# gooey-audio/libgooey

Measured on NVIDIA B200. Metric: voice-samples/sec, higher is better.
Workload: dtype f32

## Files before the change

### libgooey_b200/csrc/coop.cuh

```cuda
#pragma once
#include <climits>
#include <type_traits>
#include "wave.cuh"

namespace gd { namespace coop {
using namespace gd::wave;

constexpr unsigned FULL = 0xffffffffu;
constexpr int SP = 33;
enum { M_IDLE = 0, M_NORMAL = 1, M_TAIL = 2, M_GENERIC = 3, M_SERIAL = 4 };
enum { F_NORMAL = 1u << M_NORMAL, F_TAIL = 1u << M_TAIL, F_GENERIC = 1u << M_GENERIC, F_SERIAL = 1u << M_SERIAL, F_MEMBRANE = 1u << 8 };
struct RoundInfo { int j, nl, nv, mode; };
struct Empty {};

template <class C, int NV> struct Smem {
  typename std::conditional<C::GEO, GeoTables, Empty>::type T;
  typename C::V::Aud aud[NV];
  typename C::V::Run run[NV];
  typename C::Span2 w2[NV];
  RoundInfo ri[NV];
  unsigned wflags[2][NV];
  Lin2 lin[C::NLIN > 0 ? NV : 1][C::NLIN > 0 ? C::NLIN : 1];
  float st[C::NST][NV][SP];
};

__device__ __forceinline__ int warp_max(int x) {
#pragma unroll
  for (int d = 16; d > 0; d >>= 1) x = max(x, __shfl_xor_sync(FULL, x, d));
  return x;
}

struct TomC {
  using V = TomV;
  struct Span2 { int dummy; };
  static constexpr bool GEO = false;
  static constexpr int NLIN = 0;
  static constexpr int NST = 12;
  enum { ST_INC = 0, ST_FFWD = 0, ST_RND = 1, ST_A1 = 1, ST_FF = 2, ST_A2 = 2, ST_TP = 3, ST_FILT = 3, ST_FSP = 4, ST_RIN = 4, ST_RV = 5, ST_Y0 = 5,
         ST_ENV = 10, ST_NOISE = 11, ST_RLEV = 11 };
  static constexpr int MIN_CTAS = 2;
  static __device__ __forceinline__ int active_end(const TomV::Run&) { return 0x7fffffff; }
  template <class SM> static __device__ __forceinline__ void span_setup(SM&, int, int, const RateCtx&) {}

  template <int NV, class SM>
  static __device__ __forceinline__ void round(SM& S, const int warp, const int lane, const bool work, const float* p, const int j, int& nout, float& y,
                                               const RateCtx& rc, const unsigned rnd_idx) {
    TomAud& a = S.aud[warp];
    const TomV::Run& r = S.run[warp];
    const TomDer& d = r.d;
    const float sr = rc.sr;
    float (*st)[NV][SP] = S.st;
    const int nl = nout;
    int mode = M_IDLE, nv = 0;
    float env_l = 0.0f, noise_l = 0.0f, fade = 1.0f, mf_l = 40.0f, click = 0.0f;
    const unsigned le = (2u << lane) - 1u;
    if (work) {
      env_l = (j + lane) < r.j_env ? p[0] : r.env_final;
      noise_l = p[1];
      const float rnd_l = p[2];
      const bool complete_l = (j + lane) >= r.j_env;
      const unsigned valid = nl >= 32 ? FULL : ((1u << nl) - 1u);
      const float eb = env_l * d.bend_scaled;
      const float raw_freq = d.base_frequency * (1.0f + eb * eb);
      const unsigned m_att = __ballot_sync(FULL, env_l > 0.9f) & valid;
      const bool past0 = a.past_attack != 0u, done0 = a.main_done != 0u;
      const float ring0 = a.ring_level;
      const bool merged = a.tri_phase == a.main_sine_phase && a.tri_phase == a.mtri_phase && a.tri_phase == a.gated_sine_phase;
      const uint32_t cp = a.click_pos; const bool playing = a.click_playing != 0u;
      const bool past_l = past0 || (m_att & le) != 0u;
      const unsigned m_done = __ballot_sync(FULL, complete_l || (past_l && raw_freq < 20.0f)) & valid;
      const int first_done = done0 ? 0 : (m_done ? __ffs(m_done) - 1 : 32);
      __syncwarp();
      if (first_done == 0) {
        if (d.membrane > 0.0f && j >= r.j_env) {
          mode = M_TAIL; nv = nl;
          if (lane == 0) {
            a.main_done = 1;
            const float eb0 = r.env_final * d.bend_scaled;
            const float ff = fmaxf(fmaxf(d.base_frequency * (1.0f + eb0 * eb0), 40.0f), 20.0f);
            bp_set(a.bp, sr, ff, d.fq, 1.1f);
          }
        } else if (!(d.membrane > 0.0f) && !(ring0 > 0.0001f)) {
          mode = M_IDLE; nv = 0;
          if (lane == 0) { a.main_done = 1; a.active = 0; if (m_att & 1u) a.past_attack = 1; }
        } else { mode = M_GENERIC; nv = nl; }
      } else if (!merged) { mode = M_GENERIC; nv = nl; }
      else {
        mode = M_NORMAL; nv = first_done < nl ? first_done : nl;
        fade = (past_l && raw_freq < 40.0f) ? (raw_freq - 20.0f) / (40.0f - 20.0f) : 1.0f;
        mf_l = fmaxf(raw_freq, 40.0f);
        if (playing) { const uint32_t idx = cp + (uint32_t)lane; if (idx < 64u) click = c_tom_impulse[idx]; }
        if (lane == 0) {
          if ((m_att & (nv >= 32 ? FULL : ((1u << nv) - 1u))) != 0u) a.past_attack = 1;
          if (playing) { const uint32_t c2 = min(64u, cp + (uint32_t)nv); a.click_pos = c2; if (c2 >= 64u) a.click_playing = 0; }
        }
        st[ST_INC][warp][lane] = mf_l / sr;
        st[ST_FF][warp][lane] = fmaxf(mf_l, 20.0f);
      }
      if (mode == M_NORMAL || mode == M_GENERIC) st[ST_RND][warp][lane] = rnd_l;
      if (mode == M_GENERIC) { st[ST_ENV][warp][lane] = env_l; st[ST_NOISE][warp][lane] = noise_l; }
      if (lane == 0) {
        S.ri[warp].nv = nv; S.ri[warp].mode = mode;
      }
    }
    if (lane == 0) S.wflags[rnd_idx & 1u][warp] = mode == M_IDLE ? 0u : ((1u << mode) | ((d.membrane > 0.0f && mode != M_GENERIC) ? F_MEMBRANE : 0u));
    __syncthreads();
    const unsigned fl = __reduce_or_sync(FULL, lane < NV ? S.wflags[rnd_idx & 1u][lane] : 0u);
    if (fl & (F_NORMAL | F_GENERIC)) {
      if (warp == 0 && (fl & F_NORMAL)) {
        const int vv = lane < NV ? lane : 0;
        const bool on = lane < NV && S.ri[vv].mode == M_NORMAL;
        const int n_v = on ? S.ri[vv].nv : 0;
        TomAud& b = S.aud[vv];
        float ph = b.tri_phase, fx = b.fixed_sine_phase, rph = b.rand_phase, rcu = b.rand_current, rtg = b.rand_target;
        const float inc_fixed = 190.0f / sr, inc_rand = S.run[vv].d.rand_freq / sr;
        const float fq = S.run[vv].d.fq;
        float lf = b.bp.last_freq;
        bool qg_ok = fabsf(fq - b.bp.last_q) < 0.001f && fabsf(1.1f - b.bp.last_gain) < 0.001f;
        unsigned mask = 0u;
        const int nmax = warp_max(n_v);
        const float* r_inc = &st[ST_INC][vv][0]; const float* r_rnd = &st[ST_RND][vv][0]; const float* r_ff = &st[ST_FF][vv][0];
        float* w_tp = &st[ST_TP][vv][0]; float* w_fsp = &st[ST_FSP][vv][0]; float* w_rv = &st[ST_RV][vv][0];
        for (int n0 = 0; n0 < nmax; n0 += 8) {
          float inc[8], rnd[8], ffn[8];
#pragma unroll
          for (int k = 0; k < 8; k++) { inc[k] = r_inc[n0 + k]; rnd[k] = r_rnd[n0 + k]; ffn[k] = r_ff[n0 + k]; }
#pragma unroll
          for (int k = 0; k < 8; k++) {
            if (n0 + k < n_v) {
              w_tp[n0 + k] = ph; w_fsp[n0 + k] = fx;
              ph += inc[k]; if (ph >= 1.0f) ph -= 1.0f;
              fx += inc_fixed; if (fx >= 1.0f) fx -= 1.0f;
              const float prev = rph;
              rph += inc_rand; if (rph >= 1.0f) rph -= 1.0f;
              const bool wrap = rph < prev;
              rcu = wrap ? rtg : rcu; rtg = wrap ? rnd[k] : rtg;
              w_rv[n0 + k] = rcu + (rtg - rcu) * rph;
              const bool upd = !(fabsf(ffn[k] - lf) < 0.01f && qg_ok);
              lf = upd ? ffn[k] : lf; qg_ok = qg_ok || upd;
              mask |= upd ? (1u << (n0 + k)) : 0u;
            }
          }
        }
        if (on) {
          b.tri_phase = b.main_sine_phase = b.mtri_phase = b.gated_sine_phase = ph;
          b.fixed_sine_phase = fx; b.rand_phase = rph; b.rand_current = rcu; b.rand_target = rtg;
          b.bp.last_freq = lf;
          if (mask) { b.bp.last_q = fq; b.bp.last_gain = 1.1f; }
          S.ri[vv].nl = (int)mask;
        }
      }
      if (warp == (NV > 1 ? 1 : 0) && (fl & F_GENERIC)) {
        const int vv = lane < NV ? lane : 0;
        if (lane < NV && S.ri[vv].mode == M_GENERIC) {
          TomAud& b = S.aud[vv];
          const TomV::Run& rr = S.run[vv];
          const int jv = S.ri[vv].j, n_v = S.ri[vv].nv;
          int got = n_v;
          for (int n = 0; n < n_v; n++) {
            TomFront f; f.env = st[ST_ENV][vv][n]; f.noise = st[ST_NOISE][vv][n]; f.rnd = st[ST_RND][vv][n];
            const float yy = tom_back(b, rr.d, f, (jv + n) >= rr.j_env, rc);
            st[ST_TP][vv][n] = yy;
            if (!b.active) { got = n + 1; break; }
          }
          S.ri[vv].nv = got;
        }
      }
      __syncthreads();
    }
    float filtered = 0.0f;
    if (fl & F_NORMAL) {
      if (mode == M_NORMAL) {
        const float tp = st[ST_TP][warp][lane], fsp = st[ST_FSP][warp][lane], rand_value = st[ST_RV][warp][lane];
        const float ffl = st[ST_FF][warp][lane];
        const unsigned mask = (unsigned)S.ri[warp].nl;
        const float click_out = click * 1.1f;
        const float tri_out = a.tri_enabled ? tri_wave(tp) * 0.5f : 0.0f;
        const float us = unit_sine(tp);
        const float main_sine = us * 0.5f;
        const float mtri = tri_wave(tp) * 0.5f;
        const float fixed_sine = unit_sine(fsp) * 0.5f;
        const float noise = noise_l * 0.2f;
        const float noise_combined = (noise + rand_value) * 0.4f;
        const float gated = d.tone < 99.0f ? us * 0.2f : 0.0f;
        const float ch1 = main_sine * fixed_sine, ch2 = mtri + noise_combined, ch3 = noise_combined + gated;
        const float morph_out = ch1 * d.w1 + ch2 * d.w2 + ch3 * d.w3;
        const float x = click_out + tri_out + morph_out;
        float b0 = a.bp.b0, b1 = a.bp.b1, b2 = a.bp.b2, a1 = a.bp.a1, a2 = a.bp.a2;
        const float x1c = a.bp.x1, x2c = a.bp.x2;
        if (mask) {
          Biquad spec;
          bp_compute(spec, sr, ffl, d.fq, 1.1f);
          const unsigned m = mask & le;
          const int src = m ? 31 - __clz(m) : 0;
          const float sb0 = __shfl_sync(FULL, spec.b0, src), sb1 = __shfl_sync(FULL, spec.b1, src), sb2 = __shfl_sync(FULL, spec.b2, src);
          const float sa1 = __shfl_sync(FULL, spec.a1, src), sa2 = __shfl_sync(FULL, spec.a2, src);
          if (m) { b0 = sb0; b1 = sb1; b2 = sb2; a1 = sa1; a2 = sa2; }
        }
        float xm1 = __shfl_up_sync(FULL, x, 1), xm2 = __shfl_up_sync(FULL, x, 2);
        if (lane == 0) { xm1 = x1c; xm2 = x2c; } else if (lane == 1) xm2 = x1c;
        const float ffwd = b0 * x + b1 * xm1 + b2 * xm2;
        __syncwarp();
        st[ST_FFWD][warp][lane] = ffwd; st[ST_A1][warp][lane] = a1; st[ST_A2][warp][lane] = a2;
        if (lane == nv - 1) { Biquad& o = a.bp; o.b0 = b0; o.b1 = b1; o.b2 = b2; o.a1 = a1; o.a2 = a2; o.x1 = x; o.x2 = xm1; }
      }
      __syncthreads();
      if (warp == 0) {
        const int vv = lane < NV ? lane : 0;
        const bool on = lane < NV && S.ri[vv].mode == M_NORMAL;
        const int n_v = on ? S.ri[vv].nv : 0;
        float y1 = S.aud[vv].bp.y1, y2 = S.aud[vv].bp.y2;
        const int nmax = warp_max(n_v);
        const float* r_f = &st[ST_FFWD][vv][0]; const float* r_a1 = &st[ST_A1][vv][0]; const float* r_a2 = &st[ST_A2][vv][0];
        float* w_y = &st[ST_FILT][vv][0];
        for (int n0 = 0; n0 < nmax; n0 += 8) {
          float f[8], c1[8], c2[8], o[8];
#pragma unroll
          for (int k = 0; k < 8; k++) { f[k] = r_f[n0 + k]; c1[k] = r_a1[n0 + k]; c2[k] = r_a2[n0 + k]; }
#pragma unroll
          for (int k = 0; k < 8; k++) {
            o[k] = 0.0f;
            if (n0 + k < n_v) {
              const float out = f[k] - c1[k] * y1 - c2[k] * y2;
              y2 = y1; y1 = out;
              o[k] = fabsf(out) < 1e-15f ? 0.0f : out;
            }
          }
#pragma unroll
          for (int k = 0; k < 8; k++) if (n0 + k < n_v) w_y[n0 + k] = o[k];
        }
        if (on) { S.aud[vv].bp.y1 = y1; S.aud[vv].bp.y2 = y2; }
      }
      __syncthreads();
      if (mode == M_NORMAL) filtered = st[ST_FILT][warp][lane];
    }
    float mem_out = 0.0f, rlev = 0.0f;
    if (fl & F_MEMBRANE) {
      if ((mode == M_NORMAL || mode == M_TAIL) && d.membrane > 0.0f) {
        const float mi = mode == M_NORMAL ? filtered * env_l : 0.0f;
        const float u1 = __shfl_up_sync(FULL, mi, 1), u2 = __shfl_up_sync(FULL, mi, 2);
        float ffw[5], xp[5];
#pragma unroll
        for (int f = 0; f < 5; f++) {
          const Biquad& m = a.mem[f];
          const float xm1 = lane == 0 ? m.x1 : u1, xm2 = lane == 0 ? m.x2 : (lane == 1 ? m.x1 : u2);
          ffw[f] = m.b0 * mi + m.b1 * xm1 + m.b2 * xm2;
          xp[f] = xm1;
        }
        __syncwarp();
#pragma unroll
        for (int f = 0; f < 5; f++) {
          st[ST_Y0 + f][warp][lane] = ffw[f];
          if (lane == nv - 1) { a.mem[f].x1 = mi; a.mem[f].x2 = xp[f]; }
        }
      }
      __syncthreads();
      {
        const int q = warp * 32 + lane;
        const int f = q / NV, vv = q - f * NV;
        if (f < 5) {
          const int m = S.ri[vv].mode;
          const bool on = (m == M_NORMAL || m == M_TAIL) && S.run[vv].d.membrane > 0.0f;
          const int n_v = on ? S.ri[vv].nv : 0;
          const Biquad& bq = S.aud[vv].mem[f];
          const float a1 = bq.a1, a2 = bq.a2;
          float y1 = bq.y1, y2 = bq.y2;
          float* row = &st[ST_Y0 + f][vv][0];
          for (int n0 = 0; n0 < n_v; n0 += 8) {
            float in[8], o[8];
#pragma unroll
            for (int k = 0; k < 8; k++) in[k] = row[n0 + k];
#pragma unroll
            for (int k = 0; k < 8; k++) {
              o[k] = 0.0f;
              if (n0 + k < n_v) {
                const float out = in[k] - a1 * y1 - a2 * y2;
                y2 = y1; y1 = out;
                o[k] = fabsf(out) < 1e-15f ? 0.0f : out;
              }
            }
#pragma unroll
            for (int k = 0; k < 8; k++) if (n0 + k < n_v) row[n0 + k] = o[k];
          }
          if (on) { Biquad& o = S.aud[vv].mem[f]; o.y1 = y1; o.y2 = y2; }
        }
      }
      __syncthreads();
      if ((mode == M_NORMAL || mode == M_TAIL) && d.membrane > 0.0f) {
        float acc = 0.0f;
#pragma unroll
        for (int i = 0; i < 5; i++) acc += st[ST_Y0 + i][warp][lane];
        mem_out = w_tanh(acc);
        st[ST_RIN][warp][lane] = fabsf(mem_out) * 0.001f;
      }
      __syncthreads();
      if (warp == NV - 1) {
        const int vv = lane < NV ? lane : 0;
        const int m = S.ri[vv].mode;
        const bool on = lane < NV && (m == M_NORMAL || m == M_TAIL) && S.run[vv].d.membrane > 0.0f;
        const int n_v = on ? S.ri[vv].nv : 0;
        float ring = S.aud[vv].ring_level;
        if (m == M_TAIL) {
          int dead = -1;
          const float* r_in = &st[ST_RIN][vv][0]; float* w_lev = &st[ST_RLEV][vv][0];
          for (int n0 = 0; n0 < n_v && dead < 0; n0 += 8) {
            float in[8], lev[8];
#pragma unroll
            for (int k = 0; k < 8; k++) in[k] = r_in[n0 + k];
#pragma unroll
            for (int k = 0; k < 8; k++) {
              lev[k] = 0.0f;
              if (n0 + k < n_v && dead < 0) {
                if (!(ring > 0.0001f)) dead = n0 + k;
                else { ring = ring * 0.999f + in[k]; lev[k] = ring; }
              }
            }
#pragma unroll
            for (int k = 0; k < 8; k++) if (n0 + k < n_v) w_lev[n0 + k] = lev[k];
          }
          if (on && dead >= 0) { S.ri[vv].nv = dead; S.aud[vv].active = 0; }
        } else {
          const float* r_in = &st[ST_RIN][vv][0];
          for (int n0 = 0; n0 < n_v; n0 += 8) {
            float in[8];
#pragma unroll
            for (int k = 0; k < 8; k++) in[k] = r_in[n0 + k];
#pragma unroll
            for (int k = 0; k < 8; k++) if (n0 + k < n_v) ring = ring * 0.999f + in[k];
          }
        }
        if (on) S.aud[vv].ring_level = ring;
      }
      __syncthreads();
      if (mode == M_TAIL) rlev = st[ST_RLEV][warp][lane];
    }
    if (mode == M_NORMAL) {
      const float dry_gain = 1.0f - d.mm;
      const float dry = filtered * env_l;
      const float fs = dry * dry_gain + mem_out * d.mm;
      y = fs * fade * 0.7f * d.vol;
      nout = nv;
    } else if (mode == M_TAIL) {
      const float fd = rlev >= 0.005f ? 1.0f : (rlev <= 0.0001f ? 0.0f : (rlev - 0.0001f) / (0.005f - 0.0001f));
      y = mem_out * d.mm * fd * 0.7f * d.vol;
      nout = S.ri[warp].nv;
    } else if (mode == M_GENERIC) {
      y = st[ST_TP][warp][lane];
      nout = S.ri[warp].nv;
    } else nout = 0;
  }
};

template <class C, int NV>
__global__ void __launch_bounds__(NV * 32, C::MIN_CTAS) coop_kernel(const VoiceLaunch L) {
  using V = typename C::V; using Span = typename V::Span; using Aud = typename V::Aud;
  constexpr int WC = sizeof(typename V::Ctl) / 4;
  constexpr int WA = sizeof(Aud) / 4;
  extern __shared__ __align__(16) unsigned char coop_smem_raw[];
  Smem<C, NV>& S = *reinterpret_cast<Smem<C, NV>*>(coop_smem_raw);
  const int lane = threadIdx.x & 31, warp = threadIdx.x >> 5;
  if constexpr (C::GEO) geo_tables_init(S.T, L.rc, threadIdx.x, NV * 32);
  const int v = blockIdx.x * NV + warp;
  const bool alive = v < L.n && L.mode[v] == 0;
  const int sv = alive ? (L.slots ? (int)L.slots[v] : v) : 0;
  Aud& a = S.aud[warp];
  typename V::Run& run = S.run[warp];
  const Span* spans = nullptr;
  uint32_t ns = 0, cur = 0xffffffffu;
  bool ready = false;
  int next_j0 = 0x7fffffff;
  float* out = nullptr;
  const float* planes = nullptr;
  {
    uint32_t* aw = reinterpret_cast<uint32_t*>(&a);
    for (int w = lane; w < WA; w += 32) aw[w] = alive ? L.state[(size_t)(WC + w) * L.n_pad + sv] : 0u;
  }
  if (alive) {
    spans = reinterpret_cast<const Span*>(L.spans) + L.span_off[v];
    ns = L.n_spans[v];
    cur = L.span_cursor[v];
    if (cur != 0xffffffffu && lane == 0) V::span_resume(spans[cur], run);
    next_j0 = cur + 1u < ns ? spans[cur + 1u].j0 : 0x7fffffff;
    const long long row = L.rows ? (long long)L.rows[v] : (long long)(L.row0 + v);
    out = L.out + row * L.stride;
    planes = L.planes + (size_t)v * L.pitch;
  }
  if (lane == 0) S.ri[warp] = RoundInfo{0, 0, 0, M_IDLE};
  __syncthreads();
  const int c1 = L.chunk0 + min(L.chunk_frames, L.frames - L.chunk0);
  int j = L.chunk0;
  float pn[V::NPL];
  int pj = -1;
#pragma unroll
  for (int q = 0; q < V::NPL; q++) pn[q] = 0.0f;
  for (unsigned rnd_idx = 0;; rnd_idx++) {
    const bool more = alive && j < c1;
    bool work = false;
    int nl = 0;
    float p[V::NPL];
#pragma unroll
    for (int q = 0; q < V::NPL; q++) p[q] = 0.0f;
    if (more) {
      while (j == next_j0) {
        cur += 1u;
        if (lane == 0) V::span_begin(a, spans[cur], run, L.rc.sr);
        __syncwarp();
        ready = false;
        next_j0 = cur + 1u < ns ? spans[cur + 1u].j0 : 0x7fffffff;
      }
      const int span_end = min(next_j0, c1);
      const int act_end = min(span_end, C::active_end(run));
      if (cur == 0xffffffffu || !V::is_active(a, run, j) || j >= act_end) {
        for (int k = j + lane; k < span_end; k += 32) out[k] = 0.0f;
        j = span_end;
      } else {
        if (!ready) { __syncwarp(); C::span_setup(S, warp, lane, L.rc); __syncwarp(); ready = true; }
        nl = min(32, act_end - j);
        if (pj == j) {
#pragma unroll
          for (int q = 0; q < V::NPL; q++) { const float t = __shfl_sync(FULL, pn[q], nl - 1); p[q] = lane < nl ? pn[q] : t; }
        } else {
          const int jj = j + min(lane, nl - 1);
#pragma unroll
          for (int q = 0; q < V::NPL; q++) p[q] = planes[(size_t)q * L.plane_stride + (jj - L.chunk0)];
        }
        work = true;
        pj = j + nl;
        if (pj < c1) {
          const int jn = min(pj + lane, c1 - 1);
#pragma unroll
          for (int q = 0; q < V::NPL; q++) pn[q] = planes[(size_t)q * L.plane_stride + (jn - L.chunk0)];
        }
      }
    }
    __syncwarp();
    if (lane == 0) S.ri[warp] = RoundInfo{j, nl, nl, work ? M_NORMAL : M_IDLE};
    if (!__syncthreads_or(more ? 1 : 0)) break;
    float y = 0.0f;
    int nout = nl;
    C::template round<NV>(S, warp, lane, work, p, j, nout, y, L.rc, rnd_idx);
    if (work) {
      if (lane < nout) out[j + lane] = y;
      j += nout;
    }
  }
  __syncthreads();
  if (alive) {
    const uint32_t* aw = reinterpret_cast<const uint32_t*>(&a);
    for (int w = lane; w < WA; w += 32) L.state[(size_t)(WC + w) * L.n_pad + sv] = aw[w];
    if (lane == 0) L.span_cursor[v] = cur;
  }
}

} }
```

### libgooey_b200/csrc/gooey_b200.cu

```cuda
#include <mutex>
#include <memory>
#include "pool.cuh"
#include "patch.h"
#include "halfband_design.h"

namespace gh {

std::string& last_error() { static thread_local std::string e; return e; }
std::atomic<uint64_t> g_launches{0};
static float g_last_kernel_ms = 0.0f;
std::map<std::string, KernelStat>& kernel_stats() { static std::map<std::string, KernelStat> m; return m; }
std::mutex& kernel_stats_mutex() { static std::mutex m; return m; }

ClockTable& clock_table(float sr) {
  static std::mutex mu;
  static std::map<uint32_t, ClockTable*> tables;
  std::lock_guard<std::mutex> lk(mu);
  uint32_t key; memcpy(&key, &sr, 4);
  auto it = tables.find(key);
  if (it == tables.end()) {
    ClockTable* t = new ClockTable();
    t->dt = 1.0 / (double)sr;
    it = tables.emplace(key, t).first;
  }
  return *it->second;
}

static const int g_conn_env = setenv("CUDA_DEVICE_MAX_CONNECTIONS", "32", 0);

static std::mutex g_dev_mutex;
static std::vector<char> g_dev_ready;

static int device_count() {
  int n = 0;
  if (cudaGetDeviceCount(&n) != cudaSuccess) { cudaGetLastError(); return 0; }
  return n;
}

static void use_device(int device) {
  int n = device_count();
  if (n <= 0) throw CudaError("no CUDA device visible: libgooey_b200 has no CPU fallback");
  if (device < 0 || device >= n) throw CudaError("device index out of range");
  GH_CUDA(cudaSetDevice(device));
  std::lock_guard<std::mutex> lk(g_dev_mutex);
  if ((int)g_dev_ready.size() < n) g_dev_ready.resize(n, 0);
  if (!g_dev_ready[device]) {
    float hb[8];
    gd::design_halfband8(hb);
    GH_CUDA(cudaMemcpyToSymbol(gd::c_hb, hb, sizeof hb));
    {
      static float inv_sq[gd::INV_SQ_N];
      for (int k = 0; k < gd::INV_SQ_N; k++) { volatile float fi = (float)(2 * k + 1); volatile float sq = fi * fi; inv_sq[k] = 1.0f / sq; }
      GH_CUDA(cudaMemcpyToSymbol(gd::c_inv_sq, inv_sq, sizeof inv_sq));
    }
    double mf[128];
    for (int n = 0; n < 128; n++) mf[n] = 440.0 * pow(2.0, ((double)n - 69.0) / 12.0);
    GH_CUDA(cudaMemcpyToSymbol(gd::c_midi_freq, mf, sizeof mf));
    g_dev_ready[device] = 1;
  }
}

struct VoiceBank {
  TypeRunner<gd::KickV> kicks;
  TypeRunner<gd::SnareV> snares;
  TypeRunner<gd::HatV> hats;
  TypeRunner<gd::TomV> toms;
  TypeRunner<gd::BassV> basses;
  TypeRunner<gd::PolyV> polys;
  TypeRunner<gd::GranV> grans;
  void reset() { kicks.reset(); snares.reset(); hats.reset(); toms.reset(); basses.reset(); polys.reset(); grans.reset(); }
  int create(const GooeyVoicePatch& p, float sr) {
    switch (p.instrument) {
      case GOOEY_INSTRUMENT_KICK: { gd::KickState s; init_from_patch(s, p, sr); return kicks.pool.alloc(s); }
      case GOOEY_INSTRUMENT_SNARE: { gd::SnareState s; init_from_patch(s, p, sr); return snares.pool.alloc(s); }
      case GOOEY_INSTRUMENT_HIHAT: { gd::HatState s; init_from_patch(s, p, sr); return hats.pool.alloc(s); }
      case GOOEY_INSTRUMENT_TOM: { gd::TomState s; init_from_patch(s, p, sr); return toms.pool.alloc(s); }
      case GOOEY_INSTRUMENT_BASS: { gd::BassState s; init_from_patch(s, p, sr); return basses.pool.alloc(s); }
      case GOOEY_B200_VOICE_POLY: { gd::PolyState s; memset(&s, 0, sizeof s); gd::poly_init(s, p.params, sr); return polys.pool.alloc(s); }
      case GOOEY_B200_VOICE_GRANULATOR: { gd::GranState s; memset(&s, 0, sizeof s); gd::gran_init(s, sr); return grans.pool.alloc(s); }
      default: return -1;
    }
  }
  void set_mod(const float* planes, long long pitch, int frame0) {
    kicks.mod_planes = snares.mod_planes = hats.mod_planes = toms.mod_planes = basses.mod_planes = planes;
    kicks.mod_pitch = snares.mod_pitch = hats.mod_pitch = toms.mod_pitch = basses.mod_pitch = pitch;
    kicks.mod_frame0 = snares.mod_frame0 = hats.mod_frame0 = toms.mod_frame0 = basses.mod_frame0 = frame0;
  }
  void add(uint32_t type, uint32_t slot, uint32_t row, const std::vector<gd::VoiceEvent>& ev, const std::vector<gd::ModRoute>* routes = nullptr) {
    switch (type) {
      case GOOEY_INSTRUMENT_KICK: kicks.add(slot, row, ev, routes); break;
      case GOOEY_INSTRUMENT_SNARE: snares.add(slot, row, ev, routes); break;
      case GOOEY_INSTRUMENT_HIHAT: hats.add(slot, row, ev, routes); break;
      case GOOEY_INSTRUMENT_TOM: toms.add(slot, row, ev, routes); break;
      case GOOEY_INSTRUMENT_BASS: basses.add(slot, row, ev, routes); break;
      case GOOEY_B200_VOICE_POLY: polys.add(slot, row, ev); break;
      case GOOEY_B200_VOICE_GRANULATOR: grans.add(slot, row, ev); break;
    }
  }
  void release(uint32_t type, int slot) {
    switch (type) {
      case GOOEY_INSTRUMENT_KICK: kicks.pool.release(slot); break;
      case GOOEY_INSTRUMENT_SNARE: snares.pool.release(slot); break;
      case GOOEY_INSTRUMENT_HIHAT: hats.pool.release(slot); break;
      case GOOEY_INSTRUMENT_TOM: toms.pool.release(slot); break;
      case GOOEY_INSTRUMENT_BASS: basses.pool.release(slot); break;
      case GOOEY_B200_VOICE_POLY: polys.pool.release(slot); break;
      case GOOEY_B200_VOICE_GRANULATOR: grans.pool.release(slot); break;
    }
  }
  void launch(cudaStream_t parent, cudaEvent_t start, const gd::RateCtx& rc, const double* tt, int frames, float* out, long long stride) {
    kicks.launch(parent, start, rc, tt, frames, out, stride);
    snares.launch(parent, start, rc, tt, frames, out, stride);
    hats.launch(parent, start, rc, tt, frames, out, stride);
    toms.launch(parent, start, rc, tt, frames, out, stride);
    basses.launch(parent, start, rc, tt, frames, out, stride);
    polys.launch(parent, start, rc, tt, frames, out, stride);
    grans.launch(parent, start, rc, tt, frames, out, stride);
  }
  void collect_stats() { kicks.collect_stats(); snares.collect_stats(); hats.collect_stats(); toms.collect_stats(); }
  int chunk_frames(int frames) const { return TypeRunner<gd::KickV>::chunk_of(frames); }
  void wait_chunk(cudaStream_t s, int i) { kicks.wait_chunk(s, i); snares.wait_chunk(s, i); hats.wait_chunk(s, i); toms.wait_chunk(s, i); basses.wait_chunk(s, i); polys.wait_chunk(s, i); grans.wait_chunk(s, i); }
};

}

using namespace gh;

struct GooeyVoiceBatch {
  int device = 0;
  float sr = 44100.0f;
  gd::RateCtx rc;
  cudaStream_t stream = nullptr, copy_stream = nullptr;
  cudaEvent_t ev0 = nullptr, ev1 = nullptr;
  uint32_t n = 0;
  uint32_t k = 0;
  gh::ClockWindow clock;
  std::vector<uint8_t> vtype;
  std::vector<uint32_t> vslot;
  std::vector<std::vector<gd::VoiceEvent>> pending;
  VoiceBank bank;
  DevBuf<float> d_out;
  DevBuf<int16_t> d_pcm;
  ~GooeyVoiceBatch() {
    if (ev0) cudaEventDestroy(ev0);
    if (ev1) cudaEventDestroy(ev1);
    if (stream) cudaStreamDestroy(stream);
    if (copy_stream) cudaStreamDestroy(copy_stream);
  }
};

namespace gh {

static void voice_batch_render_impl(GooeyVoiceBatch* b, uint32_t frames, float* out_dev, size_t stride) {
  use_device(b->device);
  cudaStream_t st = b->stream;
  if ((uint64_t)b->k + frames >= 0xffffffffull) throw std::runtime_error("engine clock index overflow");
  const double* tt = b->clock.view(clock_table(b->sr), b->k, (uint64_t)b->k + frames, st);
  b->bank.reset();
  std::vector<gd::VoiceEvent> now, later;
  for (uint32_t v = 0; v < b->n; v++) {
    auto& ev = b->pending[v];
    std::stable_sort(ev.begin(), ev.end(), [](const gd::VoiceEvent& a, const gd::VoiceEvent& c) { return a.frame < c.frame; });
    now.clear(); later.clear();
    for (auto& e : ev) { if (e.frame < frames) now.push_back(e); else { e.frame -= frames; later.push_back(e); } }
    b->bank.add(b->vtype[v], b->vslot[v], v, now);
    ev = later;
  }
  GH_CUDA(cudaEventRecord(b->ev0, st));
  b->bank.launch(st, b->ev0, b->rc, tt, (int)frames, out_dev, (long long)stride);
  GH_CUDA(cudaEventRecord(b->ev1, st));
  b->k += frames;
}

}

#define GOOEY_TRY try {
#define GOOEY_CATCH                                                              \
  } catch (const gh::CudaError& e) { gh::set_error(e.what());                    \
    return std::string(e.what()).find("no CUDA device") != std::string::npos ? GOOEY_E_NO_DEVICE : GOOEY_E_CUDA; \
  } catch (const std::exception& e) { gh::set_error(e.what()); return GOOEY_E_INVALID; }

extern "C" {

const char* gooey_b200_last_error(void) { return gh::last_error().c_str(); }
int gooey_b200_device_count(void) { return gh::device_count(); }
uint64_t gooey_b200_launch_count(void) { return gh::g_launches.load(); }
float gooey_b200_last_kernel_ms(void) { return gh::g_last_kernel_ms; }
int gooey_b200_kernel_stat(const char* kernel, uint64_t* launches, double* total_ms, double* voice_frames) {
  if (!kernel) return GOOEY_E_INVALID;
  std::lock_guard<std::mutex> lk(gh::kernel_stats_mutex());
  auto it = gh::kernel_stats().find(kernel);
  gh::KernelStat k = it == gh::kernel_stats().end() ? gh::KernelStat() : it->second;
  if (launches) *launches = k.launches;
  if (total_ms) *total_ms = k.ms;
  if (voice_frames) *voice_frames = k.voice_frames;
  return GOOEY_E_OK;
}
const char* gooey_b200_kernel_stat_names(void) {
  static thread_local std::string names;
  std::lock_guard<std::mutex> lk(gh::kernel_stats_mutex());
  names.clear();
  for (const auto& kv : gh::kernel_stats()) { if (!names.empty()) names += ';'; names += kv.first; }
  return names.c_str();
}
void gooey_b200_kernel_stats_reset(void) { std::lock_guard<std::mutex> lk(gh::kernel_stats_mutex()); gh::kernel_stats().clear(); }

int gooey_voice_batch_new(float sample_rate, uint32_t n_voices, const GooeyVoicePatch* patches, int device, GooeyVoiceBatch** out_batch) {
  GOOEY_TRY
  if (!out_batch || (!patches && n_voices)) { set_error("null argument"); return GOOEY_E_INVALID; }
  *out_batch = nullptr;
  if (!(sample_rate > 0.0f)) { set_error("sample_rate must be > 0"); return GOOEY_E_INVALID; }
  use_device(device);
  std::unique_ptr<GooeyVoiceBatch> b(new GooeyVoiceBatch);
  b->device = device; b->sr = sample_rate; b->n = n_voices;
  b->rc = gd::make_rate_ctx(sample_rate);
  GH_CUDA(cudaStreamCreateWithFlags(&b->stream, cudaStreamNonBlocking));
  GH_CUDA(cudaStreamCreateWithFlags(&b->copy_stream, cudaStreamNonBlocking));
  GH_CUDA(cudaEventCreate(&b->ev0));
  GH_CUDA(cudaEventCreate(&b->ev1));
  b->vtype.resize(n_voices); b->vslot.resize(n_voices); b->pending.resize(n_voices);
  for (uint32_t v = 0; v < n_voices; v++) {
    int slot = b->bank.create(patches[v], sample_rate);
    if (slot < 0) { set_error("unsupported instrument id in voice patch"); return GOOEY_E_INVALID; }
    b->vtype[v] = (uint8_t)patches[v].instrument;
    b->vslot[v] = (uint32_t)slot;
  }
  *out_batch = b.release();
  return GOOEY_E_OK;
  GOOEY_CATCH
}

void gooey_voice_batch_free(GooeyVoiceBatch* b) {
  if (!b) return;
  cudaSetDevice(b->device);
  cudaDeviceSynchronize();
  delete b;
}

int gooey_voice_batch_trigger(GooeyVoiceBatch* b, uint32_t voice, uint32_t frame, float velocity) {
  GOOEY_TRY
  if (!b || voice >= b->n) { set_error("bad batch/voice"); return GOOEY_E_INVALID; }
  b->pending[voice].push_back(make_event(frame, gd::EV_TRIGGER, 0, velocity));
  return GOOEY_E_OK;
  GOOEY_CATCH
}

int gooey_voice_batch_trigger_all(GooeyVoiceBatch* b, uint32_t frame, const float* velocities) {
  GOOEY_TRY
  if (!b) { set_error("null batch"); return GOOEY_E_INVALID; }
  for (uint32_t v = 0; v < b->n; v++) b->pending[v].push_back(make_event(frame, gd::EV_TRIGGER, 0, velocities ? velocities[v] : 1.0f));
  return GOOEY_E_OK;
  GOOEY_CATCH
}

int gooey_voice_batch_set_param(GooeyVoiceBatch* b, uint32_t voice, uint32_t frame, uint32_t param, float value, int snap) {
  GOOEY_TRY
  if (!b || voice >= b->n) { set_error("bad batch/voice"); return GOOEY_E_INVALID; }
  bool known = ffi_param_to_events(b->vtype[voice], param, value,
                                   [&](uint32_t kind, uint32_t p, float v) { b->pending[voice].push_back(make_event(frame, kind, p, v)); });
  if (known && snap) b->pending[voice].push_back(make_event(frame, gd::EV_SNAP, 0, 0.0f));
  return GOOEY_E_OK;
  GOOEY_CATCH
}

int gooey_voice_batch_render_device(GooeyVoiceBatch* b, uint32_t frames, float* out_dev, size_t stride) {
  GOOEY_TRY
  if (!b || !out_dev || stride < frames) { set_error("bad arguments"); return GOOEY_E_INVALID; }
  voice_batch_render_impl(b, frames, out_dev, stride);
  GH_CUDA(cudaStreamSynchronize(b->stream));
  GH_CUDA(cudaEventElapsedTime(&gh::g_last_kernel_ms, b->ev0, b->ev1));
  b->bank.collect_stats();
  return GOOEY_E_OK;
  GOOEY_CATCH
}

int gooey_voice_batch_render(GooeyVoiceBatch* b, uint32_t frames, float* out_host) {
  GOOEY_TRY
  if (!b || !out_host) { set_error("bad arguments"); return GOOEY_E_INVALID; }
  use_device(b->device);
  const size_t stride = (frames + 3) & ~(size_t)3;
  b->d_out.alloc((size_t)b->n * stride);
  voice_batch_render_impl(b, frames, b->d_out.p, stride);
  const uint32_t chunk = (uint32_t)b->bank.chunk_frames((int)frames);
  int ci = 0;
  for (uint32_t c0 = 0; c0 < frames; c0 += chunk, ci++) {
    const uint32_t nf = std::min(chunk, frames - c0);
    b->bank.wait_chunk(b->copy_stream, ci);
    GH_CUDA(cudaMemcpy2DAsync(out_host + c0, (size_t)frames * 4, b->d_out.p + c0, stride * 4, (size_t)nf * 4, b->n, cudaMemcpyDeviceToHost, b->copy_stream));
  }
  GH_CUDA(cudaStreamSynchronize(b->copy_stream));
  GH_CUDA(cudaStreamSynchronize(b->stream));
  GH_CUDA(cudaEventElapsedTime(&gh::g_last_kernel_ms, b->ev0, b->ev1));
  b->bank.collect_stats();
  return GOOEY_E_OK;
  GOOEY_CATCH
}

}

#include "engine_api.cuh"
#include "rs_api.cuh"
#include "loops_api.cuh"
#include <sys/syscall.h>
#include <unistd.h>

extern "C" {

int gooey_voice_batch_render_pcm16(GooeyVoiceBatch* b, uint32_t frames, int16_t* out_host) {
  GOOEY_TRY
  if (!b || !out_host) { set_error("bad arguments"); return GOOEY_E_INVALID; }
  use_device(b->device);
  const size_t stride = (frames + 3) & ~(size_t)3;
  b->d_out.alloc((size_t)b->n * stride);
  b->d_pcm.alloc((size_t)b->n * stride);
  voice_batch_render_impl(b, frames, b->d_out.p, stride);
  const uint32_t chunk = (uint32_t)b->bank.chunk_frames((int)frames);
  int ci = 0;
  for (uint32_t c0 = 0; c0 < frames; c0 += chunk, ci++) {
    const uint32_t nf = std::min(chunk, frames - c0);
    b->bank.wait_chunk(b->copy_stream, ci);
    gd::quantize_pcm16_kernel<<<dim3((nf + 1023) / 1024, b->n), 256, 0, b->copy_stream>>>(b->d_out.p, (long long)stride, b->d_pcm.p, (long long)stride, (int)c0, (int)nf);
    g_launches.fetch_add(1, std::memory_order_relaxed);
    GH_CUDA(cudaGetLastError());
    GH_CUDA(cudaMemcpy2DAsync(out_host + c0, (size_t)frames * 2, b->d_pcm.p + c0, stride * 2, (size_t)nf * 2, b->n, cudaMemcpyDeviceToHost, b->copy_stream));
  }
  GH_CUDA(cudaStreamSynchronize(b->copy_stream));
  GH_CUDA(cudaStreamSynchronize(b->stream));
  GH_CUDA(cudaEventElapsedTime(&gh::g_last_kernel_ms, b->ev0, b->ev1));
  b->bank.collect_stats();
  return GOOEY_E_OK;
  GOOEY_CATCH
}

void* gooey_b200_host_alloc(size_t bytes, int device, int* out_numa_node) {
  if (out_numa_node) *out_numa_node = -1;
  if (bytes == 0) return nullptr;
  try { use_device(device); } catch (const std::exception& ex) { set_error(ex.what()); return nullptr; }
  int node = -1;
  char bus[32] = {0};
  if (cudaDeviceGetPCIBusId(bus, sizeof bus, device) == cudaSuccess) {
    for (char* c = bus; *c; c++) *c = (char)tolower(*c);
    const std::string path = std::string("/sys/bus/pci/devices/") + bus + "/numa_node";
    if (FILE* f = fopen(path.c_str(), "r")) { if (fscanf(f, "%d", &node) != 1) node = -1; fclose(f); }
  } else cudaGetLastError();
  bool bound = false;
#ifdef SYS_set_mempolicy
  if (node >= 0 && node < 1024) {
    unsigned long mask[16] = {0};
    mask[node / (8 * sizeof(unsigned long))] |= 1ul << (node % (8 * sizeof(unsigned long)));
    bound = syscall(SYS_set_mempolicy, 1 , mask, (unsigned long)(sizeof mask * 8)) == 0;
  }
#endif
  void* p = nullptr;
  const cudaError_t e = cudaHostAlloc(&p, bytes, cudaHostAllocPortable);
  if (e == cudaSuccess) memset(p, 0, bytes);
  if (e == cudaSuccess) {
    void* d = nullptr;
    const size_t chunk = (size_t)64 << 20;
    if (cudaMalloc(&d, std::min(chunk, bytes)) == cudaSuccess) {
      cudaMemset(d, 0, std::min(chunk, bytes));
      for (size_t off = 0; off < bytes; off += chunk)
        cudaMemcpyAsync((char*)p + off, d, std::min(chunk, bytes - off), cudaMemcpyDeviceToHost, 0);
      cudaDeviceSynchronize();
      cudaFree(d);
    }
    cudaGetLastError();
  }
#ifdef SYS_set_mempolicy
  if (bound) syscall(SYS_set_mempolicy, 0 , nullptr, 0ul);
#endif
  if (e != cudaSuccess) { cudaGetLastError(); set_error("cudaHostAlloc failed"); return nullptr; }
  if (out_numa_node) *out_numa_node = bound ? node : -1;
  return p;
}
void gooey_b200_host_free(void* p) { if (p) cudaFreeHost(p); }

}

namespace gh {
__global__ void math_selftest_kernel(int kind, const float* x, const float* y, float* out, uint32_t n) {
  uint32_t i = blockIdx.x * blockDim.x + threadIdx.x;
  if (i >= n) return;
  float r;
  switch (kind) {
    case 0: r = gm::g_powf(x[i], y[i]); break;
    case 1: r = gm::g_sinf(x[i]); break;
    case 2: r = gm::g_cosf(x[i]); break;
    case 3: r = gm::g_expf(x[i]); break;
    case 4: r = gd::hash_noise((uint64_t)x[i]); break;
    case 5: r = gd::max_curve(x[i], y[i]); break;
    case 6: r = gm::g_tanhf(x[i]); break;
    case 7: r = gm::g_tanf(x[i]); break;
    case 8: r = gm::g_expm1f(x[i]); break;
    case 9: r = gm::g_sinf_fast(x[i]); break;
    case 10: r = gm::g_div_by(x[i], y[i], 1.0f / y[i]); break;
    default: r = 0.0f;
  }
  out[i] = r;
}
}

extern "C" int gooey_b200_selftest_math(int kind, const float* x_host, const float* y_host, float* out_host, uint32_t n, int device) {
  GOOEY_TRY
  use_device(device);
  DevBuf<float> dx, dy, dout;
  dx.upload(x_host, n, 0);
  dy.upload(y_host ? y_host : x_host, n, 0);
  dout.alloc(n);
  gh::math_selftest_kernel<<<(n + 255) / 256, 256>>>(kind, dx.p, dy.p, dout.p, n);
  g_launches.fetch_add(1);
  GH_CUDA(cudaGetLastError());
  GH_CUDA(cudaMemcpy(out_host, dout.p, (size_t)n * 4, cudaMemcpyDeviceToHost));
  return GOOEY_E_OK;
  GOOEY_CATCH
}
```

### libgooey_b200/csrc/pool.cuh

```cuda
#pragma once
#include <algorithm>
#include <atomic>
#include <map>
#include <type_traits>
#include <set>
#include <mutex>
#include "device_rt.h"
#include "wave.cuh"
#include "coop.cuh"
#include "gran_wave.cuh"
#include "bass_wave.cuh"
#include "../../include/gooey_batch.h"

namespace gh {

extern std::atomic<uint64_t> g_launches;

struct KernelStat { uint64_t launches = 0; double ms = 0.0; double voice_frames = 0.0; };
std::map<std::string, KernelStat>& kernel_stats();
std::mutex& kernel_stats_mutex();

__global__ void scatter_words_kernel(uint32_t* __restrict__ dst, long long cap, const uint32_t* __restrict__ src, const uint32_t* __restrict__ slots,
                                     int n, int words) {
  const int k = blockIdx.x * blockDim.x + threadIdx.x;
  if (k >= n) return;
  const uint32_t s = slots[k];
  for (int w = 0; w < words; w++) dst[(long long)w * cap + s] = src[(long long)w * n + k];
}

template <class S> struct Pool {
  static_assert(sizeof(S) % 4 == 0, "state must be whole 32-bit words");
  static constexpr int W = sizeof(S) / 4;
  DevBuf<uint32_t> d;
  int cap = 0, count = 0;
  std::vector<int> free_list;
  std::vector<std::pair<int, S>> pending;

  int alloc(const S& init) {
    int slot;
    if (!free_list.empty()) { slot = free_list.back(); free_list.pop_back(); } else slot = count++;
    pending.emplace_back(slot, init);
    return slot;
  }
  void release(int slot) {
    for (size_t i = 0; i < pending.size(); i++) if (pending[i].first == slot) { pending.erase(pending.begin() + i); break; }
    free_list.push_back(slot);
  }
  void flush(cudaStream_t st) {
    if (count > cap) {
      int ncap = std::max(pad32(count), cap * 2);
      if (((ncap / 32) & 1) == 0) ncap += 32;
      DevBuf<uint32_t> nd;
      nd.alloc((size_t)W * ncap);
      GH_CUDA(cudaMemsetAsync(nd.p, 0, (size_t)W * ncap * 4, st));
      if (cap > 0) GH_CUDA(cudaMemcpy2DAsync(nd.p, (size_t)ncap * 4, d.p, (size_t)cap * 4, (size_t)cap * 4, W, cudaMemcpyDeviceToDevice, st));
      GH_CUDA(cudaStreamSynchronize(st));
      std::swap(d.p, nd.p); std::swap(d.n, nd.n);
      cap = ncap;
    }
    if (pending.empty()) return;
    const int n = (int)pending.size();
    std::vector<uint32_t> words((size_t)W * n), slots(n);
    for (int k = 0; k < n; k++) {
      slots[k] = (uint32_t)pending[k].first;
      const uint32_t* w = reinterpret_cast<const uint32_t*>(&pending[k].second);
      for (int i = 0; i < W; i++) words[(size_t)i * n + k] = w[i];
    }
    DevBuf<uint32_t> dw, ds;
    dw.upload(words.data(), words.size(), st);
    ds.upload(slots.data(), slots.size(), st);
    scatter_words_kernel<<<(n + 127) / 128, 128, 0, st>>>(d.p, cap, dw.p, ds.p, n, W);
    g_launches.fetch_add(1);
    GH_CUDA(cudaGetLastError());
    GH_CUDA(cudaStreamSynchronize(st));
    pending.clear();
    pending.shrink_to_fit();
  }
};

inline gd::VoiceEvent make_event(uint32_t frame, uint32_t kind, uint32_t param, float value, uint32_t aux = 0) {
  gd::VoiceEvent e; e.frame = frame; e.kind = (uint16_t)kind; e.param = (uint16_t)param; e.value = value; e.aux = aux;
  return e;
}

struct ClockTable {
  static constexpr uint64_t CK = 65536;
  double dt = 0.0;
  std::vector<double> ckpt;
  std::mutex mu;
  void fill(uint64_t k0, size_t n, double* out) {
    std::lock_guard<std::mutex> lk(mu);
    if (ckpt.empty()) ckpt.push_back(0.0);
    const uint64_t need = k0 / CK;
    while (ckpt.size() <= need) { double t = ckpt.back(); for (uint64_t i = 0; i < CK; i++) t += dt; ckpt.push_back(t); }
    double t = ckpt[need];
    for (uint64_t k = need * CK; k < k0; k++) t += dt;
    for (size_t i = 0; i < n; i++) { out[i] = t; t += dt; }
  }
};
struct ClockWindow {
  DevBuf<double> d;
  std::vector<double> h;
  uint64_t k0 = 0; size_t n = 0;
  const double* view(ClockTable& T, uint64_t kmin, uint64_t kmax, cudaStream_t st) {
    if (kmin > 0) kmin -= 1;
    if (!(n && kmin >= k0 && kmax < k0 + n)) {
      const size_t want = (size_t)(kmax - kmin + 1);
      const size_t cap = std::max<size_t>((want + 8191) & ~(size_t)8191, 1u << 16);
      if (d.n < cap) { GH_CUDA(cudaStreamSynchronize(st)); d.alloc(cap); }
      h.resize(want);
      T.fill(kmin, want, h.data());
      GH_CUDA(cudaMemcpyAsync(d.p, h.data(), want * sizeof(double), cudaMemcpyHostToDevice, st));
      GH_CUDA(cudaStreamSynchronize(st));
      k0 = kmin; n = want;
    }
    return d.p - k0;
  }
};
ClockTable& clock_table(float sr);

enum class Back { Wave, Coop, Serial };
constexpr int COOP_FROM = 4096;
constexpr int COOP_NV = 16;
constexpr int SERIAL_FROM = 12288;
inline bool serial_backend() { const char* e = getenv("GOOEY_B200_BACKEND"); return e && strcmp(e, "serial") == 0; }
template <class V> inline Back choose_back(int cnt) {
  if (serial_backend()) return Back::Serial;
  if (std::is_same<V, gd::TomV>::value) return cnt >= COOP_FROM ? Back::Coop : Back::Wave;
  return cnt >= SERIAL_FROM ? Back::Serial : Back::Wave;
}
template <class V> struct WaveOf;
template <> struct WaveOf<gd::KickV> { using W = gd::wave::KickW; static constexpr const char* name = "wave_kernel<KickW>"; };
template <> struct WaveOf<gd::SnareV> { using W = gd::wave::SnareW; static constexpr const char* name = "wave_kernel<SnareW>"; };
template <> struct WaveOf<gd::HatV> { using W = gd::wave::HatW; static constexpr const char* name = "wave_kernel<HatW>"; };
template <> struct WaveOf<gd::TomV> { using W = gd::wave::TomW; static constexpr const char* name = "wave_kernel<TomW>"; };

inline void coop_launch(int cnt, cudaStream_t s, const gd::VoiceLaunch& L) {
  using SM = gd::coop::Smem<gd::coop::TomC, COOP_NV>;
  auto kernel = gd::coop::coop_kernel<gd::coop::TomC, COOP_NV>;
  static std::mutex mu;
  static std::set<int> done;
  int dev = 0;
  cudaGetDevice(&dev);
  {
    std::lock_guard<std::mutex> lk(mu);
    if (done.insert(dev).second) {
      GH_CUDA(cudaFuncSetAttribute((const void*)kernel, cudaFuncAttributeMaxDynamicSharedMemorySize, (int)sizeof(SM)));
      GH_CUDA(cudaFuncSetAttribute((const void*)kernel, cudaFuncAttributePreferredSharedMemoryCarveout, (int)cudaSharedmemCarveoutMaxShared));
    }
  }
  kernel<<<(cnt + COOP_NV - 1) / COOP_NV, COOP_NV * 32, sizeof(SM), s>>>(L);
}

template <class K> inline void same_carveout(K kernel) {
  static std::mutex mu;
  static std::set<std::pair<int, const void*>> done;
  int dev = 0;
  cudaGetDevice(&dev);
  std::lock_guard<std::mutex> lk(mu);
  if (done.insert({dev, (const void*)kernel}).second)
    GH_CUDA(cudaFuncSetAttribute((const void*)kernel, cudaFuncAttributePreferredSharedMemoryCarveout, (int)cudaSharedmemCarveoutMaxShared));
}
#define GH_LAUNCH(kernel, grid, block, stream, ...) do { same_carveout(kernel); kernel<<<grid, block, 0, stream>>>(__VA_ARGS__); } while (0)

constexpr int CHUNK_FRAMES = 8192;
template <class V> struct TypeRunner {
  using State = typename V::State;
  Pool<State> pool;
  std::vector<uint32_t> slots, rows, ev_begin, span_off;
  std::vector<gd::VoiceEvent> ev_flat;
  std::vector<gd::ModRoute> routes_flat; std::vector<uint32_t> route_begin;
  DevBuf<gd::ModRoute> d_routes; DevBuf<uint32_t> d_route_begin;
  const float* mod_planes = nullptr; long long mod_pitch = 0; int mod_frame0 = 0;
  DevBuf<uint32_t> d_slots, d_rows, d_ev_begin, d_span_off, d_n_spans, d_span_cursor;
  DevBuf<gd::VoiceEvent> d_events;
  DevBuf<uint8_t> d_mode, d_spans;
  DevBuf<float> d_planes[2];
  cudaStream_t sB = nullptr, sC = nullptr, sS = nullptr;
  cudaEvent_t evA = nullptr, evB[2] = {nullptr, nullptr}, evC[2] = {nullptr, nullptr}, evDoneC = nullptr, evDoneS = nullptr;
  std::vector<cudaEvent_t> evT0, evT1;
  std::vector<double> timed_units;
  std::vector<cudaEvent_t> evChunk;
  int launched_chunks = 0;
  const char* backend_name = "back_kernel";
  static int chunk_of(int frames) { return std::min(CHUNK_FRAMES, (frames + 31) & ~31); }
  void wait_chunk(cudaStream_t s, int i) {
    if (n() == 0) return;
    if (launched_chunks == 0) { GH_CUDA(cudaStreamWaitEvent(s, evDoneC, 0)); return; }
    GH_CUDA(cudaStreamWaitEvent(s, evDoneS, 0));
    GH_CUDA(cudaStreamWaitEvent(s, evChunk[std::min(i, std::abs(launched_chunks) - 1)], 0));
  }

  int n() const { return (int)slots.size(); }
  void reset() { slots.clear(); rows.clear(); ev_flat.clear(); ev_begin.clear(); ev_begin.push_back(0); span_off.clear(); span_off.push_back(0);
                 routes_flat.clear(); route_begin.clear(); route_begin.push_back(0); }
  void add(uint32_t slot, uint32_t out_row, const std::vector<gd::VoiceEvent>& events, const std::vector<gd::ModRoute>* routes = nullptr) {
    slots.push_back(slot); rows.push_back(out_row);
    if (routes) routes_flat.insert(routes_flat.end(), routes->begin(), routes->end());
    route_begin.push_back((uint32_t)routes_flat.size());
    uint32_t distinct = 0, last = 0xffffffffu;
    for (const auto& e : events) { if (e.frame != last) { distinct++; last = e.frame; } }
    ev_flat.insert(ev_flat.end(), events.begin(), events.end());
    ev_begin.push_back((uint32_t)ev_flat.size());
    span_off.push_back(span_off.back() + distinct + 1);
  }
  void ensure_streams() {
    if (sC) return;
    GH_CUDA(cudaStreamCreateWithFlags(&sB, cudaStreamNonBlocking));
    GH_CUDA(cudaStreamCreateWithFlags(&sC, cudaStreamNonBlocking));
    GH_CUDA(cudaStreamCreateWithFlags(&sS, cudaStreamNonBlocking));
    cudaEvent_t* evs[] = {&evA, &evB[0], &evB[1], &evC[0], &evC[1], &evDoneC, &evDoneS};
    for (auto e : evs) GH_CUDA(cudaEventCreateWithFlags(e, cudaEventDisableTiming));
  }
  ~TypeRunner() {
    cudaEvent_t evs[] = {evA, evB[0], evB[1], evC[0], evC[1], evDoneC, evDoneS};
    for (auto e : evs) if (e) cudaEventDestroy(e);
    for (auto e : evChunk) cudaEventDestroy(e);
    for (auto e : evT0) cudaEventDestroy(e);
    for (auto e : evT1) cudaEventDestroy(e);
    if (sB) cudaStreamDestroy(sB);
    if (sC) cudaStreamDestroy(sC);
    if (sS) cudaStreamDestroy(sS);
  }
  void collect_stats() {
    const char* name = backend_name;
    if (launched_chunks <= 0) return;
    std::lock_guard<std::mutex> lk(kernel_stats_mutex());
    KernelStat& k = kernel_stats()[name];
    for (int i = 0; i < launched_chunks; i++) {
      float ms = 0.0f;
      if (cudaEventElapsedTime(&ms, evT0[i], evT1[i]) != cudaSuccess) { cudaGetLastError(); continue; }
      k.launches++; k.ms += ms; k.voice_frames += timed_units[i];
    }
    launched_chunks = -launched_chunks;
  }
  void launch(cudaStream_t parent, cudaEvent_t start, const gd::RateCtx& rc, const double* tt, int frames, float* out, long long stride) {
    const int cnt = n();
    launched_chunks = 0;
    if (cnt == 0 || frames <= 0) return;
    ensure_streams();
    GH_CUDA(cudaStreamWaitEvent(sC, start, 0));
    pool.flush(sC);
    d_slots.upload(slots.data(), slots.size(), sC);
    d_rows.upload(rows.data(), rows.size(), sC);
    if (ev_flat.empty()) ev_flat.push_back(make_event(0xffffffffu, 0xffff, 0, 0.0f));
    d_events.upload(ev_flat.data(), ev_flat.size(), sC);
    d_ev_begin.upload(ev_begin.data(), ev_begin.size(), sC);
    gd::VoiceLaunch L;
    memset(&L, 0, sizeof L);
    L.state = pool.d.p; L.n = cnt; L.n_pad = pool.cap;
    L.slots = d_slots.p; L.rows = d_rows.p; L.row0 = 0;
    L.events = d_events.p; L.ev_begin = d_ev_begin.p; L.tt = tt; L.frames = frames; L.out = out; L.stride = stride; L.rc = rc;
    const bool modulated = !routes_flat.empty() && mod_planes;
    if (modulated) {
      d_routes.upload(routes_flat.data(), routes_flat.size(), sC);
      d_route_begin.upload(route_begin.data(), route_begin.size(), sC);
      L.routes = d_routes.p; L.route_begin = d_route_begin.p; L.mod_planes = mod_planes; L.mod_pitch = mod_pitch; L.mod_frame0 = mod_frame0;
    }
    if constexpr (V::FAST) {
      using Span = typename V::Span;
      d_span_off.upload(span_off.data(), span_off.size(), sC);
      d_n_spans.alloc(cnt); d_span_cursor.alloc(cnt); d_mode.alloc(cnt);
      d_spans.alloc((size_t)span_off.back() * sizeof(Span));
      const int chunk = chunk_of(frames);
      const int rows_pad = pad32(cnt);
      const size_t plane_floats = (size_t)rows_pad * chunk;
      d_planes[0].alloc(plane_floats * V::NPL); d_planes[1].alloc(plane_floats * V::NPL);
      L.mode = d_mode.p; L.spans = d_spans.p; L.span_off = d_span_off.p; L.n_spans = d_n_spans.p; L.span_cursor = d_span_cursor.p;
      L.plane_stride = (long long)plane_floats; L.pitch = chunk;
      GH_LAUNCH((gd::plan_kernel<V>), (cnt + 63) / 64, 64, sC, L);
      g_launches.fetch_add(1, std::memory_order_relaxed);
      GH_CUDA(cudaGetLastError());
      GH_CUDA(cudaEventRecord(evA, sC));
      GH_CUDA(cudaStreamWaitEvent(sB, evA, 0));
      GH_CUDA(cudaStreamWaitEvent(sS, evA, 0));
      GH_LAUNCH((gd::slow_kernel<V, 32>), (cnt + 31) / 32, 32, sS, L);
      g_launches.fetch_add(1, std::memory_order_relaxed);
      GH_CUDA(cudaGetLastError());
      GH_CUDA(cudaEventRecord(evDoneS, sS));
      const Back back = choose_back<V>(cnt);
      int i = 0;
      for (int c0 = 0; c0 < frames; c0 += chunk, i++) {
        const int b = i & 1;
        L.chunk0 = c0; L.chunk_frames = std::min(chunk, frames - c0);
        L.planes = d_planes[b].p;
        if (i >= 2) GH_CUDA(cudaStreamWaitEvent(sB, evC[b], 0));
        const int bpv = (L.chunk_frames + 255) / 256;
        GH_LAUNCH((gd::front_kernel<V, 256>), (unsigned)((size_t)cnt * bpv), 256, sB, L, bpv);
        GH_CUDA(cudaGetLastError());
        GH_CUDA(cudaEventRecord(evB[b], sB));
        GH_CUDA(cudaStreamWaitEvent(sC, evB[b], 0));
        if ((int)evT0.size() <= i) { cudaEvent_t e0, e1; GH_CUDA(cudaEventCreate(&e0)); GH_CUDA(cudaEventCreate(&e1)); evT0.push_back(e0); evT1.push_back(e1); timed_units.push_back(0.0); }
        timed_units[i] = (double)cnt * L.chunk_frames;
        GH_CUDA(cudaEventRecord(evT0[i], sC));
        switch (back) {
          case Back::Coop:
            if constexpr (std::is_same<V, gd::TomV>::value) coop_launch(cnt, sC, L);
            backend_name = "coop_kernel<TomC>";
            break;
          case Back::Wave:
            GH_LAUNCH((gd::wave::wave_kernel<typename WaveOf<V>::W>), cnt, 32, sC, L);
            backend_name = WaveOf<V>::name;
            break;
          case Back::Serial:
            GH_LAUNCH((gd::back_kernel<V, 32>), (cnt + 31) / 32, 32, sC, L);
            backend_name = "back_kernel";
            break;
        }
        GH_CUDA(cudaGetLastError());
        GH_CUDA(cudaEventRecord(evT1[i], sC));
        GH_CUDA(cudaEventRecord(evC[b], sC));
        if ((int)evChunk.size() <= i) { cudaEvent_t e; GH_CUDA(cudaEventCreateWithFlags(&e, cudaEventDisableTiming)); evChunk.push_back(e); }
        GH_CUDA(cudaEventRecord(evChunk[i], sC));
        g_launches.fetch_add(2, std::memory_order_relaxed);
      }
      launched_chunks = i;
      GH_CUDA(cudaEventRecord(evDoneC, sC));
      GH_CUDA(cudaStreamWaitEvent(parent, evDoneC, 0));
      GH_CUDA(cudaStreamWaitEvent(parent, evDoneS, 0));
      if (getenv("GOOEY_B200_TRACE_TYPES")) {
        cudaEvent_t t0, t1, t2;
        cudaEventCreate(&t0); cudaEventCreate(&t1); cudaEventCreate(&t2);
        cudaEventRecord(t1, sC); cudaEventRecord(t2, sS);
        GH_CUDA(cudaStreamSynchronize(sC)); GH_CUDA(cudaStreamSynchronize(sS));
        std::vector<uint8_t> mode(cnt);
        GH_CUDA(cudaMemcpy(mode.data(), d_mode.p, cnt, cudaMemcpyDeviceToHost));
        int slow = 0; for (uint8_t m : mode) slow += m != 0;
        float ms_all = 0.0f;
        cudaEventElapsedTime(&ms_all, evT0[0], t1);
        float ms_slow_end = 0.0f;
        cudaEventElapsedTime(&ms_slow_end, evT0[0], t2);
        fprintf(stderr, "[gooey trace]   %s: %d voices x %d frames, %d on the per-sample path; back ends done %.1f ms, per-sample kernel done %.1f ms after the first back-end launch\n",
                backend_name, cnt, frames, slow, ms_all, ms_slow_end);
        cudaEventDestroy(t0); cudaEventDestroy(t1); cudaEventDestroy(t2);
      }
    } else {
      if constexpr (std::is_same<V, gd::GranV>::value) {
        GH_LAUNCH((gd::gran_wave_kernel<4>), (cnt + 3) / 4, 128, sC, L);
      } else if (std::is_same<V, gd::BassV>::value && !modulated) {
        const bool ttrace = getenv("GOOEY_B200_TRACE_TYPES") != nullptr;
        cudaEvent_t t0 = nullptr, t1 = nullptr;
        if (ttrace) { cudaEventCreate(&t0); cudaEventCreate(&t1); cudaEventRecord(t0, sC); }
        GH_LAUNCH((gd::bass_wave_kernel<2>), (cnt + 1) / 2, 64, sC, L);
        if (ttrace) {
          cudaEventRecord(t1, sC); GH_CUDA(cudaStreamSynchronize(sC));
          float ms = 0.0f; cudaEventElapsedTime(&ms, t0, t1);
          fprintf(stderr, "[gooey trace]   bass_wave_kernel: %d voices x %d frames, %.1f ms\n", cnt, frames, ms);
          cudaEventDestroy(t0); cudaEventDestroy(t1);
        }
      } else if (cnt <= 148 * 32 * 4) GH_LAUNCH((gd::slow_kernel<V, 32>), (cnt + 31) / 32, 32, sC, L);
      else GH_LAUNCH((gd::slow_kernel<V, 128>), (cnt + 127) / 128, 128, sC, L);
      g_launches.fetch_add(1, std::memory_order_relaxed);
      GH_CUDA(cudaGetLastError());
      GH_CUDA(cudaEventRecord(evDoneC, sC));
      GH_CUDA(cudaStreamWaitEvent(parent, evDoneC, 0));
    }
  }
};

}
```

Baseline: 8.403 billion.

## Pipeline tom coop kernel into multi-round staggered stages across specialized warps

Restructures the cooperative tom kernel from one synchronous round, where a few warps run serial recurrences while the others wait, into a software pipeline of depth four. Each stage runs on its own warp: phase/random, filter-update mask, bandpass recurrence, five membrane biquads and ring level, plus a dedicated generic warp. A ring buffer of round info lets each stage work on a different in-flight block. The voices per block drop from 16 to 8, and the coop backend is now chosen by the total drum voice count rather than the tom count alone. This adds shared-memory staging and pipeline fill/drain bookkeeping, with a risk of ordering bugs around generic and tail modes.

```diff
diff --git a/libgooey_b200/csrc/coop.cuh b/libgooey_b200/csrc/coop.cuh
--- a/libgooey_b200/csrc/coop.cuh
+++ b/libgooey_b200/csrc/coop.cuh
@@ -8,21 +8,10 @@
 
 constexpr unsigned FULL = 0xffffffffu;
 constexpr int SP = 33;
-enum { M_IDLE = 0, M_NORMAL = 1, M_TAIL = 2, M_GENERIC = 3, M_SERIAL = 4 };
-enum { F_NORMAL = 1u << M_NORMAL, F_TAIL = 1u << M_TAIL, F_GENERIC = 1u << M_GENERIC, F_SERIAL = 1u << M_SERIAL, F_MEMBRANE = 1u << 8 };
-struct RoundInfo { int j, nl, nv, mode; };
-struct Empty {};
-
-template <class C, int NV> struct Smem {
-  typename std::conditional<C::GEO, GeoTables, Empty>::type T;
-  typename C::V::Aud aud[NV];
-  typename C::V::Run run[NV];
-  typename C::Span2 w2[NV];
-  RoundInfo ri[NV];
-  unsigned wflags[2][NV];
-  Lin2 lin[C::NLIN > 0 ? NV : 1][C::NLIN > 0 ? C::NLIN : 1];
-  float st[C::NST][NV][SP];
-};
+constexpr int DEPTH = 4;
+constexpr int RING = 8;
+enum { M_IDLE = 0, M_NORMAL = 1, M_TAIL = 2, M_GENERIC = 3 };
+struct RoundInfo { int j, nl, nv, mode; unsigned mask; };
 
 __device__ __forceinline__ int warp_max(int x) {
 #pragma unroll
@@ -32,99 +21,52 @@
 
 struct TomC {
   using V = TomV;
-  struct Span2 { int dummy; };
-  static constexpr bool GEO = false;
-  static constexpr int NLIN = 0;
-  static constexpr int NST = 12;
-  enum { ST_INC = 0, ST_FFWD = 0, ST_RND = 1, ST_A1 = 1, ST_FF = 2, ST_A2 = 2, ST_TP = 3, ST_FILT = 3, ST_FSP = 4, ST_RIN = 4, ST_RV = 5, ST_Y0 = 5,
-         ST_ENV = 10, ST_NOISE = 11, ST_RLEV = 11 };
-  static constexpr int MIN_CTAS = 2;
-  static __device__ __forceinline__ int active_end(const TomV::Run&) { return 0x7fffffff; }
-  template <class SM> static __device__ __forceinline__ void span_setup(SM&, int, int, const RateCtx&) {}
+  static constexpr int NST = 18;
+  enum { ST_INC = 0, ST_ENV = 0, ST_RND = 1, ST_FF = 2, ST_NOISE = 2,
+         ST_TP = 3, ST_FSP = 4, ST_RV = 5,
+         ST_FFWD = 6, ST_A1 = 7, ST_A2 = 8,
+         ST_FILT = 9,
+         ST_Y0 = 10,
+         ST_RIN = 15,
+         ST_RLEV = 16,
+         ST_GEN = 17 };
+  enum { W_S1 = 0, W_S2 = 1, W_S3 = 2, W_S4 = 5, W_GEN = 6, W_S1M = 7 };
+  static constexpr int MIN_WARPS = 32;
+
+  template <int NV> struct Smem {
+    TomAud aud[NV];
+    TomV::Run run[NV];
+    RoundInfo ri[RING][NV];
+    int dead_j[NV];
+    float st[NST][NV][SP];
+  };
+  struct Carry {
+    float noise, click, ff, env, fade;
+    float env_c, fade_c;
+    float dry, fade_d;
+    float pre;
+  };
 
   template <int NV, class SM>
-  static __device__ __forceinline__ void round(SM& S, const int warp, const int lane, const bool work, const float* p, const int j, int& nout, float& y,
-                                               const RateCtx& rc, const unsigned rnd_idx) {
-    TomAud& a = S.aud[warp];
-    const TomV::Run& r = S.run[warp];
-    const TomDer& d = r.d;
+  static __device__ __forceinline__ void s_half(SM& S, const int warp, const int lane, const unsigned t, const RateCtx& rc) {
     const float sr = rc.sr;
     float (*st)[NV][SP] = S.st;
-    const int nl = nout;
-    int mode = M_IDLE, nv = 0;
-    float env_l = 0.0f, noise_l = 0.0f, fade = 1.0f, mf_l = 40.0f, click = 0.0f;
-    const unsigned le = (2u << lane) - 1u;
-    if (work) {
-      env_l = (j + lane) < r.j_env ? p[0] : r.env_final;
-      noise_l = p[1];
-      const float rnd_l = p[2];
-      const bool complete_l = (j + lane) >= r.j_env;
-      const unsigned valid = nl >= 32 ? FULL : ((1u << nl) - 1u);
-      const float eb = env_l * d.bend_scaled;
-      const float raw_freq = d.base_frequency * (1.0f + eb * eb);
-      const unsigned m_att = __ballot_sync(FULL, env_l > 0.9f) & valid;
-      const bool past0 = a.past_attack != 0u, done0 = a.main_done != 0u;
-      const float ring0 = a.ring_level;
-      const bool merged = a.tri_phase == a.main_sine_phase && a.tri_phase == a.mtri_phase && a.tri_phase == a.gated_sine_phase;
-      const uint32_t cp = a.click_pos; const bool playing = a.click_playing != 0u;
-      const bool past_l = past0 || (m_att & le) != 0u;
-      const unsigned m_done = __ballot_sync(FULL, complete_l || (past_l && raw_freq < 20.0f)) & valid;
-      const int first_done = done0 ? 0 : (m_done ? __ffs(m_done) - 1 : 32);
-      __syncwarp();
-      if (first_done == 0) {
-        if (d.membrane > 0.0f && j >= r.j_env) {
-          mode = M_TAIL; nv = nl;
-          if (lane == 0) {
-            a.main_done = 1;
-            const float eb0 = r.env_final * d.bend_scaled;
-            const float ff = fmaxf(fmaxf(d.base_frequency * (1.0f + eb0 * eb0), 40.0f), 20.0f);
-            bp_set(a.bp, sr, ff, d.fq, 1.1f);
-          }
-        } else if (!(d.membrane > 0.0f) && !(ring0 > 0.0001f)) {
-          mode = M_IDLE; nv = 0;
-          if (lane == 0) { a.main_done = 1; a.active = 0; if (m_att & 1u) a.past_attack = 1; }
-        } else { mode = M_GENERIC; nv = nl; }
-      } else if (!merged) { mode = M_GENERIC; nv = nl; }
-      else {
-        mode = M_NORMAL; nv = first_done < nl ? first_done : nl;
-        fade = (past_l && raw_freq < 40.0f) ? (raw_freq - 20.0f) / (40.0f - 20.0f) : 1.0f;
-        mf_l = fmaxf(raw_freq, 40.0f);
-        if (playing) { const uint32_t idx = cp + (uint32_t)lane; if (idx < 64u) click = c_tom_impulse[idx]; }
-        if (lane == 0) {
-          if ((m_att & (nv >= 32 ? FULL : ((1u << nv) - 1u))) != 0u) a.past_attack = 1;
-          if (playing) { const uint32_t c2 = min(64u, cp + (uint32_t)nv); a.click_pos = c2; if (c2 >= 64u) a.click_playing = 0; }
-        }
-        st[ST_INC][warp][lane] = mf_l / sr;
-        st[ST_FF][warp][lane] = fmaxf(mf_l, 20.0f);
-      }
-      if (mode == M_NORMAL || mode == M_GENERIC) st[ST_RND][warp][lane] = rnd_l;
-      if (mode == M_GENERIC) { st[ST_ENV][warp][lane] = env_l; st[ST_NOISE][warp][lane] = noise_l; }
-      if (lane == 0) {
-        S.ri[warp].nv = nv; S.ri[warp].mode = mode;
-      }
-    }
-    if (lane == 0) S.wflags[rnd_idx & 1u][warp] = mode == M_IDLE ? 0u : ((1u << mode) | ((d.membrane > 0.0f && mode != M_GENERIC) ? F_MEMBRANE : 0u));
-    __syncthreads();
-    const unsigned fl = __reduce_or_sync(FULL, lane < NV ? S.wflags[rnd_idx & 1u][lane] : 0u);
-    if (fl & (F_NORMAL | F_GENERIC)) {
-      if (warp == 0 && (fl & F_NORMAL)) {
-        const int vv = lane < NV ? lane : 0;
-        const bool on = lane < NV && S.ri[vv].mode == M_NORMAL;
-        const int n_v = on ? S.ri[vv].nv : 0;
-        TomAud& b = S.aud[vv];
+    const int vv = lane < NV ? lane : 0;
+    if (warp == W_S1 || warp == W_S1M) {
+      const RoundInfo& q = S.ri[(t - 1u) & (RING - 1)][vv];
+      const bool on = lane < NV && q.mode == M_NORMAL;
+      const int n_v = on ? q.nv : 0;
+      const int nmax = warp_max(n_v);
+      TomAud& b = S.aud[vv];
+      if (nmax > 0 && warp == W_S1) {
         float ph = b.tri_phase, fx = b.fixed_sine_phase, rph = b.rand_phase, rcu = b.rand_current, rtg = b.rand_target;
         const float inc_fixed = 190.0f / sr, inc_rand = S.run[vv].d.rand_freq / sr;
-        const float fq = S.run[vv].d.fq;
-        float lf = b.bp.last_freq;
-        bool qg_ok = fabsf(fq - b.bp.last_q) < 0.001f && fabsf(1.1f - b.bp.last_gain) < 0.001f;
-        unsigned mask = 0u;
-        const int nmax = warp_max(n_v);
-        const float* r_inc = &st[ST_INC][vv][0]; const float* r_rnd = &st[ST_RND][vv][0]; const float* r_ff = &st[ST_FF][vv][0];
+        const float* r_inc = &st[ST_INC][vv][0]; const float* r_rnd = &st[ST_RND][vv][0];
         float* w_tp = &st[ST_TP][vv][0]; float* w_fsp = &st[ST_FSP][vv][0]; float* w_rv = &st[ST_RV][vv][0];
         for (int n0 = 0; n0 < nmax; n0 += 8) {
-          float inc[8], rnd[8], ffn[8];
-#pragma unroll
-          for (int k = 0; k < 8; k++) { inc[k] = r_inc[n0 + k]; rnd[k] = r_rnd[n0 + k]; ffn[k] = r_ff[n0 + k]; }
+          float inc[8], rnd[8];
+#pragma unroll
+          for (int k = 0; k < 8; k++) { inc[k] = r_inc[n0 + k]; rnd[k] = r_rnd[n0 + k]; }
 #pragma unroll
           for (int k = 0; k < 8; k++) {
             if (n0 + k < n_v) {
@@ -136,6 +78,26 @@
               const bool wrap = rph < prev;
               rcu = wrap ? rtg : rcu; rtg = wrap ? rnd[k] : rtg;
               w_rv[n0 + k] = rcu + (rtg - rcu) * rph;
+            }
+          }
+        }
+        if (on) {
+          b.tri_phase = b.main_sine_phase = b.mtri_phase = b.gated_sine_phase = ph;
+          b.fixed_sine_phase = fx; b.rand_phase = rph; b.rand_current = rcu; b.rand_target = rtg;
+        }
+      } else if (nmax > 0) {
+        const float fq = S.run[vv].d.fq;
+        float lf = b.bp.last_freq;
+        bool qg_ok = fabsf(fq - b.bp.last_q) < 0.001f && fabsf(1.1f - b.bp.last_gain) < 0.001f;
+        unsigned mask = 0u;
+        const float* r_ff = &st[ST_FF][vv][0];
+        for (int n0 = 0; n0 < nmax; n0 += 8) {
+          float ffn[8];
+#pragma unroll
+          for (int k = 0; k < 8; k++) ffn[k] = r_ff[n0 + k];
+#pragma unroll
+          for (int k = 0; k < 8; k++) {
+            if (n0 + k < n_v) {
               const bool upd = !(fabsf(ffn[k] - lf) < 0.01f && qg_ok);
               lf = upd ? ffn[k] : lf; qg_ok = qg_ok || upd;
               mask |= upd ? (1u << (n0 + k)) : 0u;
@@ -143,44 +105,200 @@
           }
         }
         if (on) {
-          b.tri_phase = b.main_sine_phase = b.mtri_phase = b.gated_sine_phase = ph;
-          b.fixed_sine_phase = fx; b.rand_phase = rph; b.rand_current = rcu; b.rand_target = rtg;
           b.bp.last_freq = lf;
           if (mask) { b.bp.last_q = fq; b.bp.last_gain = 1.1f; }
-          S.ri[vv].nl = (int)mask;
-        }
-      }
-      if (warp == (NV > 1 ? 1 : 0) && (fl & F_GENERIC)) {
-        const int vv = lane < NV ? lane : 0;
-        if (lane < NV && S.ri[vv].mode == M_GENERIC) {
-          TomAud& b = S.aud[vv];
-          const TomV::Run& rr = S.run[vv];
-          const int jv = S.ri[vv].j, n_v = S.ri[vv].nv;
-          int got = n_v;
-          for (int n = 0; n < n_v; n++) {
-            TomFront f; f.env = st[ST_ENV][vv][n]; f.noise = st[ST_NOISE][vv][n]; f.rnd = st[ST_RND][vv][n];
-            const float yy = tom_back(b, rr.d, f, (jv + n) >= rr.j_env, rc);
-            st[ST_TP][vv][n] = yy;
-            if (!b.active) { got = n + 1; break; }
-          }
-          S.ri[vv].nv = got;
-        }
-      }
-      __syncthreads();
-    }
-    float filtered = 0.0f;
-    if (fl & F_NORMAL) {
-      if (mode == M_NORMAL) {
+          S.ri[(t - 1u) & (RING - 1)][vv].mask = mask;
+        }
+      }
+    } else if (warp == W_GEN) {
+      RoundInfo& q = S.ri[(t - 1u) & (RING - 1)][vv];
+      if (lane < NV && q.mode == M_GENERIC) {
+        TomAud& b = S.aud[vv];
+        const TomV::Run& rr = S.run[vv];
+        const int jv = q.j, n_v = q.nv;
+        int got = n_v;
+        for (int n = 0; n < n_v; n++) {
+          TomFront f; f.env = st[ST_ENV][vv][n]; f.noise = st[ST_NOISE][vv][n]; f.rnd = st[ST_RND][vv][n];
+          const float yy = tom_back(b, rr.d, f, (jv + n) >= rr.j_env, rc);
+          st[ST_GEN][vv][n] = yy;
+          if (!b.active) { got = n + 1; break; }
+        }
+        q.nv = got;
+      }
+    } else if (warp == W_S2) {
+      const RoundInfo& q = S.ri[(t - 2u) & (RING - 1)][vv];
+      const bool on = lane < NV && q.mode == M_NORMAL;
+      const int n_v = on ? q.nv : 0;
+      const int nmax = warp_max(n_v);
+      if (nmax > 0) {
+        float y1 = S.aud[vv].bp.y1, y2 = S.aud[vv].bp.y2;
+        const float* r_f = &st[ST_FFWD][vv][0]; const float* r_a1 = &st[ST_A1][vv][0]; const float* r_a2 = &st[ST_A2][vv][0];
+        float* w_y = &st[ST_FILT][vv][0];
+        for (int n0 = 0; n0 < nmax; n0 += 8) {
+          float f[8], c1[8], c2[8], o[8];
+#pragma unroll
+          for (int k = 0; k < 8; k++) { f[k] = r_f[n0 + k]; c1[k] = r_a1[n0 + k]; c2[k] = r_a2[n0 + k]; }
+#pragma unroll
+          for (int k = 0; k < 8; k++) {
+            o[k] = 0.0f;
+            if (n0 + k < n_v) {
+              const float out = f[k] - c1[k] * y1 - c2[k] * y2;
+              y2 = y1; y1 = out;
+              o[k] = fabsf(out) < 1e-15f ? 0.0f : out;
+            }
+          }
+#pragma unroll
+          for (int k = 0; k < 8; k++) if (n0 + k < n_v) w_y[n0 + k] = o[k];
+        }
+        if (on) { S.aud[vv].bp.y1 = y1; S.aud[vv].bp.y2 = y2; }
+      }
+    } else if (warp >= W_S3 && warp < W_S3 + 3) {
+      const int qi = (warp - W_S3) * 32 + lane;
+      const int f = qi / NV, v3 = qi - f * NV;
+      if (f < 5) {
+        const RoundInfo& q = S.ri[(t - 3u) & (RING - 1)][v3];
+        const bool on = (q.mode == M_NORMAL || q.mode == M_TAIL) && S.run[v3].d.membrane > 0.0f;
+        const int n_v = on ? q.nv : 0;
+        if (n_v > 0) {
+          Biquad& bq = S.aud[v3].mem[f];
+          const float a1 = bq.a1, a2 = bq.a2;
+          float y1 = bq.y1, y2 = bq.y2;
+          float* row = &st[ST_Y0 + f][v3][0];
+          for (int n0 = 0; n0 < n_v; n0 += 8) {
+            float in[8], o[8];
+#pragma unroll
+            for (int k = 0; k < 8; k++) in[k] = row[n0 + k];
+#pragma unroll
+            for (int k = 0; k < 8; k++) {
+              o[k] = 0.0f;
+              if (n0 + k < n_v) {
+                const float out = in[k] - a1 * y1 - a2 * y2;
+                y2 = y1; y1 = out;
+                o[k] = fabsf(out) < 1e-15f ? 0.0f : out;
+              }
+            }
+#pragma unroll
+            for (int k = 0; k < 8; k++) if (n0 + k < n_v) row[n0 + k] = o[k];
+          }
+          bq.y1 = y1; bq.y2 = y2;
+        }
+      }
+    } else if (warp == W_S4) {
+      RoundInfo& q = S.ri[(t - 4u) & (RING - 1)][vv];
+      const bool on = lane < NV && (q.mode == M_NORMAL || q.mode == M_TAIL) && S.run[vv].d.membrane > 0.0f && q.j < S.dead_j[vv];
+      const int n_v = on ? q.nv : 0;
+      if (n_v > 0) {
+        float ring = S.aud[vv].ring_level;
+        const float* r_in = &st[ST_RIN][vv][0];
+        if (q.mode == M_TAIL) {
+          int dead = -1;
+          float* w_lev = &st[ST_RLEV][vv][0];
+          for (int n0 = 0; n0 < n_v && dead < 0; n0 += 8) {
+            float in[8], lev[8];
+#pragma unroll
+            for (int k = 0; k < 8; k++) in[k] = r_in[n0 + k];
+#pragma unroll
+            for (int k = 0; k < 8; k++) {
+              lev[k] = 0.0f;
+              if (n0 + k < n_v && dead < 0) {
+                if (!(ring > 0.0001f)) dead = n0 + k;
+                else { ring = ring * 0.999f + in[k]; lev[k] = ring; }
+              }
+            }
+#pragma unroll
+            for (int k = 0; k < 8; k++) if (n0 + k < n_v) w_lev[n0 + k] = lev[k];
+          }
+          if (dead >= 0) { q.nv = dead; S.aud[vv].active = 0; S.dead_j[vv] = q.j + dead; }
+        } else {
+          for (int n0 = 0; n0 < n_v; n0 += 8) {
+            float in[8];
+#pragma unroll
+            for (int k = 0; k < 8; k++) in[k] = r_in[n0 + k];
+#pragma unroll
+            for (int k = 0; k < 8; k++) if (n0 + k < n_v) ring = ring * 0.999f + in[k];
+          }
+        }
+        S.aud[vv].ring_level = ring;
+      }
+    }
+  }
+
+  template <int NV, class SM>
+  static __device__ __forceinline__ void p_half(SM& S, const int warp, const int lane, const unsigned t, Carry& c, float* out,
+                                                const RateCtx& rc) {
+    TomAud& a = S.aud[warp];
+    const TomDer& d = S.run[warp].d;
+    const float sr = rc.sr;
+    float (*st)[NV][SP] = S.st;
+    const unsigned le = (2u << lane) - 1u;
+    {
+      const RoundInfo& q = S.ri[(t - 4u) & (RING - 1)][warp];
+      if (q.mode == M_NORMAL) {
+        if (lane < q.nv) out[q.j + lane] = c.pre;
+      } else if (q.mode == M_TAIL) {
+        const float rlev = st[ST_RLEV][warp][lane];
+        const float fd = rlev >= 0.005f ? 1.0f : (rlev <= 0.0001f ? 0.0f : (rlev - 0.0001f) / (0.005f - 0.0001f));
+        const float y = q.j + lane < S.dead_j[warp] ? c.pre * d.mm * fd * 0.7f * d.vol : 0.0f;
+        if (lane < q.nl) out[q.j + lane] = y;
+      } else if (q.mode == M_GENERIC) {
+        if (lane < q.nv) out[q.j + lane] = st[ST_GEN][warp][lane];
+      }
+    }
+    {
+      const RoundInfo& q = S.ri[(t - 3u) & (RING - 1)][warp];
+      float mem_out = 0.0f;
+      if ((q.mode == M_NORMAL || q.mode == M_TAIL) && d.membrane > 0.0f) {
+        float acc = 0.0f;
+#pragma unroll
+        for (int i = 0; i < 5; i++) acc += st[ST_Y0 + i][warp][lane];
+        mem_out = w_tanh(acc);
+        st[ST_RIN][warp][lane] = fabsf(mem_out) * 0.001f;
+      }
+      if (q.mode == M_NORMAL) {
+        const float dry_gain = 1.0f - d.mm;
+        const float fs = c.dry * dry_gain + mem_out * d.mm;
+        c.pre = fs * c.fade_d * 0.7f * d.vol;
+      } else c.pre = mem_out;
+    }
+    __syncwarp();
+    {
+      const RoundInfo& q = S.ri[(t - 2u) & (RING - 1)][warp];
+      const float dry = q.mode == M_NORMAL ? st[ST_FILT][warp][lane] * c.env_c : 0.0f;
+      c.dry = dry; c.fade_d = c.fade_c;
+      if ((q.mode == M_NORMAL || q.mode == M_TAIL) && d.membrane > 0.0f) {
+        const float mi = dry;
+        const float u1 = __shfl_up_sync(FULL, mi, 1), u2 = __shfl_up_sync(FULL, mi, 2);
+        float ffw[5], xp[5];
+#pragma unroll
+        for (int f = 0; f < 5; f++) {
+          const Biquad& m = a.mem[f];
+          const float xm1 = lane == 0 ? m.x1 : u1, xm2 = lane == 0 ? m.x2 : (lane == 1 ? m.x1 : u2);
+          ffw[f] = m.b0 * mi + m.b1 * xm1 + m.b2 * xm2;
+          xp[f] = xm1;
+        }
+        __syncwarp();
+#pragma unroll
+        for (int f = 0; f < 5; f++) {
+          st[ST_Y0 + f][warp][lane] = ffw[f];
+          if (lane == q.nv - 1) { a.mem[f].x1 = mi; a.mem[f].x2 = xp[f]; }
+        }
+      }
+    }
+    {
+      const RoundInfo& q = S.ri[(t - 1u) & (RING - 1)][warp];
+      c.env_c = c.env; c.fade_c = c.fade;
+      if (q.mode == M_NORMAL) {
         const float tp = st[ST_TP][warp][lane], fsp = st[ST_FSP][warp][lane], rand_value = st[ST_RV][warp][lane];
-        const float ffl = st[ST_FF][warp][lane];
-        const unsigned mask = (unsigned)S.ri[warp].nl;
-        const float click_out = click * 1.1f;
+        const float ffl = c.ff;
+        const unsigned mask = q.mask;
+        const int nv = q.nv;
+        const float click_out = c.click * 1.1f;
         const float tri_out = a.tri_enabled ? tri_wave(tp) * 0.5f : 0.0f;
         const float us = unit_sine(tp);
         const float main_sine = us * 0.5f;
         const float mtri = tri_wave(tp) * 0.5f;
         const float fixed_sine = unit_sine(fsp) * 0.5f;
-        const float noise = noise_l * 0.2f;
+        const float noise = c.noise * 0.2f;
         const float noise_combined = (noise + rand_value) * 0.4f;
         const float gated = d.tone < 99.0f ? us * 0.2f : 0.0f;
         const float ch1 = main_sine * fixed_sine, ch2 = mtri + noise_combined, ch3 = noise_combined + gated;
@@ -203,163 +321,85 @@
         __syncwarp();
         st[ST_FFWD][warp][lane] = ffwd; st[ST_A1][warp][lane] = a1; st[ST_A2][warp][lane] = a2;
         if (lane == nv - 1) { Biquad& o = a.bp; o.b0 = b0; o.b1 = b1; o.b2 = b2; o.a1 = a1; o.a2 = a2; o.x1 = x; o.x2 = xm1; }
-      }
-      __syncthreads();
-      if (warp == 0) {
-        const int vv = lane < NV ? lane : 0;
-        const bool on = lane < NV && S.ri[vv].mode == M_NORMAL;
-        const int n_v = on ? S.ri[vv].nv : 0;
-        float y1 = S.aud[vv].bp.y1, y2 = S.aud[vv].bp.y2;
-        const int nmax = warp_max(n_v);
-        const float* r_f = &st[ST_FFWD][vv][0]; const float* r_a1 = &st[ST_A1][vv][0]; const float* r_a2 = &st[ST_A2][vv][0];
-        float* w_y = &st[ST_FILT][vv][0];
-        for (int n0 = 0; n0 < nmax; n0 += 8) {
-          float f[8], c1[8], c2[8], o[8];
-#pragma unroll
-          for (int k = 0; k < 8; k++) { f[k] = r_f[n0 + k]; c1[k] = r_a1[n0 + k]; c2[k] = r_a2[n0 + k]; }
-#pragma unroll
-          for (int k = 0; k < 8; k++) {
-            o[k] = 0.0f;
-            if (n0 + k < n_v) {
-              const float out = f[k] - c1[k] * y1 - c2[k] * y2;
-              y2 = y1; y1 = out;
-              o[k] = fabsf(out) < 1e-15f ? 0.0f : out;
-            }
-          }
-#pragma unroll
-          for (int k = 0; k < 8; k++) if (n0 + k < n_v) w_y[n0 + k] = o[k];
-        }
-        if (on) { S.aud[vv].bp.y1 = y1; S.aud[vv].bp.y2 = y2; }
-      }
-      __syncthreads();
-      if (mode == M_NORMAL) filtered = st[ST_FILT][warp][lane];
-    }
-    float mem_out = 0.0f, rlev = 0.0f;
-    if (fl & F_MEMBRANE) {
-      if ((mode == M_NORMAL || mode == M_TAIL) && d.membrane > 0.0f) {
-        const float mi = mode == M_NORMAL ? filtered * env_l : 0.0f;
-        const float u1 = __shfl_up_sync(FULL, mi, 1), u2 = __shfl_up_sync(FULL, mi, 2);
-        float ffw[5], xp[5];
-#pragma unroll
-        for (int f = 0; f < 5; f++) {
-          const Biquad& m = a.mem[f];
-          const float xm1 = lane == 0 ? m.x1 : u1, xm2 = lane == 0 ? m.x2 : (lane == 1 ? m.x1 : u2);
-          ffw[f] = m.b0 * mi + m.b1 * xm1 + m.b2 * xm2;
-          xp[f] = xm1;
-        }
-        __syncwarp();
-#pragma unroll
-        for (int f = 0; f < 5; f++) {
-          st[ST_Y0 + f][warp][lane] = ffw[f];
-          if (lane == nv - 1) { a.mem[f].x1 = mi; a.mem[f].x2 = xp[f]; }
-        }
-      }
-      __syncthreads();
-      {
-        const int q = warp * 32 + lane;
-        const int f = q / NV, vv = q - f * NV;
-        if (f < 5) {
-          const int m = S.ri[vv].mode;
-          const bool on = (m == M_NORMAL || m == M_TAIL) && S.run[vv].d.membrane > 0.0f;
-          const int n_v = on ? S.ri[vv].nv : 0;
-          const Biquad& bq = S.aud[vv].mem[f];
-          const float a1 = bq.a1, a2 = bq.a2;
-          float y1 = bq.y1, y2 = bq.y2;
-          float* row = &st[ST_Y0 + f][vv][0];
-          for (int n0 = 0; n0 < n_v; n0 += 8) {
-            float in[8], o[8];
-#pragma unroll
-            for (int k = 0; k < 8; k++) in[k] = row[n0 + k];
-#pragma unroll
-            for (int k = 0; k < 8; k++) {
-              o[k] = 0.0f;
-              if (n0 + k < n_v) {
-                const float out = in[k] - a1 * y1 - a2 * y2;
-                y2 = y1; y1 = out;
-                o[k] = fabsf(out) < 1e-15f ? 0.0f : out;
-              }
-            }
-#pragma unroll
-            for (int k = 0; k < 8; k++) if (n0 + k < n_v) row[n0 + k] = o[k];
-          }
-          if (on) { Biquad& o = S.aud[vv].mem[f]; o.y1 = y1; o.y2 = y2; }
-        }
-      }
-      __syncthreads();
-      if ((mode == M_NORMAL || mode == M_TAIL) && d.membrane > 0.0f) {
-        float acc = 0.0f;
-#pragma unroll
-        for (int i = 0; i < 5; i++) acc += st[ST_Y0 + i][warp][lane];
-        mem_out = w_tanh(acc);
-        st[ST_RIN][warp][lane] = fabsf(mem_out) * 0.001f;
-      }
-      __syncthreads();
-      if (warp == NV - 1) {
-        const int vv = lane < NV ? lane : 0;
-        const int m = S.ri[vv].mode;
-        const bool on = lane < NV && (m == M_NORMAL || m == M_TAIL) && S.run[vv].d.membrane > 0.0f;
-        const int n_v = on ? S.ri[vv].nv : 0;
-        float ring = S.aud[vv].ring_level;
-        if (m == M_TAIL) {
-          int dead = -1;
-          const float* r_in = &st[ST_RIN][vv][0]; float* w_lev = &st[ST_RLEV][vv][0];
-          for (int n0 = 0; n0 < n_v && dead < 0; n0 += 8) {
-            float in[8], lev[8];
-#pragma unroll
-            for (int k = 0; k < 8; k++) in[k] = r_in[n0 + k];
-#pragma unroll
-            for (int k = 0; k < 8; k++) {
-              lev[k] = 0.0f;
-              if (n0 + k < n_v && dead < 0) {
-                if (!(ring > 0.0001f)) dead = n0 + k;
-                else { ring = ring * 0.999f + in[k]; lev[k] = ring; }
-              }
-            }
-#pragma unroll
-            for (int k = 0; k < 8; k++) if (n0 + k < n_v) w_lev[n0 + k] = lev[k];
-          }
-          if (on && dead >= 0) { S.ri[vv].nv = dead; S.aud[vv].active = 0; }
-        } else {
-          const float* r_in = &st[ST_RIN][vv][0];
-          for (int n0 = 0; n0 < n_v; n0 += 8) {
-            float in[8];
-#pragma unroll
-            for (int k = 0; k < 8; k++) in[k] = r_in[n0 + k];
-#pragma unroll
-            for (int k = 0; k < 8; k++) if (n0 + k < n_v) ring = ring * 0.999f + in[k];
-          }
-        }
-        if (on) S.aud[vv].ring_level = ring;
-      }
-      __syncthreads();
-      if (mode == M_TAIL) rlev = st[ST_RLEV][warp][lane];
-    }
-    if (mode == M_NORMAL) {
-      const float dry_gain = 1.0f - d.mm;
-      const float dry = filtered * env_l;
-      const float fs = dry * dry_gain + mem_out * d.mm;
-      y = fs * fade * 0.7f * d.vol;
-      nout = nv;
-    } else if (mode == M_TAIL) {
-      const float fd = rlev >= 0.005f ? 1.0f : (rlev <= 0.0001f ? 0.0f : (rlev - 0.0001f) / (0.005f - 0.0001f));
-      y = mem_out * d.mm * fd * 0.7f * d.vol;
-      nout = S.ri[warp].nv;
-    } else if (mode == M_GENERIC) {
-      y = st[ST_TP][warp][lane];
-      nout = S.ri[warp].nv;
-    } else nout = 0;
+      } else if (q.mode == M_TAIL && lane == 0) {
+        const TomV::Run& r = S.run[warp];
+        const float eb0 = r.env_final * d.bend_scaled;
+        const float ff = fmaxf(fmaxf(d.base_frequency * (1.0f + eb0 * eb0), 40.0f), 20.0f);
+        bp_set(a.bp, sr, ff, d.fq, 1.1f);
+      }
+    }
+  }
+
+  template <int NV, class SM>
+  static __device__ __forceinline__ int stage_a(SM& S, const int warp, const int lane, const unsigned t, const float* p, const int j,
+                                                const int nl, const bool drained, Carry& c, int& mode_out, const RateCtx& rc) {
+    TomAud& a = S.aud[warp];
+    const TomV::Run& r = S.run[warp];
+    const TomDer& d = r.d;
+    const float sr = rc.sr;
+    float (*st)[NV][SP] = S.st;
+    int mode = M_IDLE, nv = 0;
+    const unsigned le = (2u << lane) - 1u;
+    const float env_l = (j + lane) < r.j_env ? p[0] : r.env_final;
+    const float noise_l = p[1];
+    const float rnd_l = p[2];
+    const bool complete_l = (j + lane) >= r.j_env;
+    const unsigned valid = nl >= 32 ? FULL : ((1u << nl) - 1u);
+    const float eb = env_l * d.bend_scaled;
+    const float raw_freq = d.base_frequency * (1.0f + eb * eb);
+    const unsigned m_att = __ballot_sync(FULL, env_l > 0.9f) & valid;
+    const bool past0 = a.past_attack != 0u, done0 = a.main_done != 0u;
+    const float ring0 = a.ring_level;
+    const bool merged = a.tri_phase == a.main_sine_phase && a.tri_phase == a.mtri_phase && a.tri_phase == a.gated_sine_phase;
+    const uint32_t cp = a.click_pos; const bool playing = a.click_playing != 0u;
+    const bool past_l = past0 || (m_att & le) != 0u;
+    const unsigned m_done = __ballot_sync(FULL, complete_l || (past_l && raw_freq < 20.0f)) & valid;
+    const int first_done = done0 ? 0 : (m_done ? __ffs(m_done) - 1 : 32);
+    __syncwarp();
+    float fade = 1.0f, mf_l = 40.0f, click = 0.0f;
+    if (first_done == 0) {
+      if (d.membrane > 0.0f && j >= r.j_env) {
+        mode = M_TAIL; nv = nl;
+        if (lane == 0) a.main_done = 1;
+      } else if (!(d.membrane > 0.0f) && !(ring0 > 0.0001f)) {
+        mode = M_IDLE; nv = 0;
+        if (lane == 0) { a.main_done = 1; a.active = 0; if (m_att & 1u) a.past_attack = 1; }
+      } else { mode = M_GENERIC; nv = nl; }
+    } else if (!merged) { mode = M_GENERIC; nv = nl; }
+    else {
+      mode = M_NORMAL; nv = first_done < nl ? first_done : nl;
+      fade = (past_l && raw_freq < 40.0f) ? (raw_freq - 20.0f) / (40.0f - 20.0f) : 1.0f;
+      mf_l = fmaxf(raw_freq, 40.0f);
+      if (playing) { const uint32_t idx = cp + (uint32_t)lane; if (idx < 64u) click = c_tom_impulse[idx]; }
+      if (lane == 0) {
+        if ((m_att & (nv >= 32 ? FULL : ((1u << nv) - 1u))) != 0u) a.past_attack = 1;
+        if (playing) { const uint32_t c2 = min(64u, cp + (uint32_t)nv); a.click_pos = c2; if (c2 >= 64u) a.click_playing = 0; }
+      }
+      st[ST_INC][warp][lane] = mf_l / sr;
+      st[ST_FF][warp][lane] = fmaxf(mf_l, 20.0f);
+      st[ST_RND][warp][lane] = rnd_l;
+    }
+    if (mode == M_GENERIC) {
+      if (!drained) return -1;
+      st[ST_ENV][warp][lane] = env_l; st[ST_NOISE][warp][lane] = noise_l; st[ST_RND][warp][lane] = rnd_l;
+    }
+    c.noise = noise_l; c.click = click; c.ff = fmaxf(mf_l, 20.0f); c.env = env_l; c.fade = fade;
+    if (lane == 0) S.ri[t & (RING - 1)][warp] = RoundInfo{j, nl, nv, mode, 0u};
+    mode_out = mode;
+    return nv;
   }
 };
 
 template <class C, int NV>
-__global__ void __launch_bounds__(NV * 32, C::MIN_CTAS) coop_kernel(const VoiceLaunch L) {
+__global__ void __launch_bounds__(NV * 32, C::MIN_WARPS / NV) coop_kernel(const VoiceLaunch L) {
+  static_assert(NV > C::W_GEN && NV > C::W_S1M && 5 * NV <= 3 * 32, "the S-half warp roles need NV warps");
   using V = typename C::V; using Span = typename V::Span; using Aud = typename V::Aud;
+  using SM = typename C::template Smem<NV>;
   constexpr int WC = sizeof(typename V::Ctl) / 4;
   constexpr int WA = sizeof(Aud) / 4;
   extern __shared__ __align__(16) unsigned char coop_smem_raw[];
-  Smem<C, NV>& S = *reinterpret_cast<Smem<C, NV>*>(coop_smem_raw);
+  SM& S = *reinterpret_cast<SM*>(coop_smem_raw);
   const int lane = threadIdx.x & 31, warp = threadIdx.x >> 5;
-  if constexpr (C::GEO) geo_tables_init(S.T, L.rc, threadIdx.x, NV * 32);
   const int v = blockIdx.x * NV + warp;
   const bool alive = v < L.n && L.mode[v] == 0;
   const int sv = alive ? (L.slots ? (int)L.slots[v] : v) : 0;
@@ -367,7 +407,6 @@
   typename V::Run& run = S.run[warp];
   const Span* spans = nullptr;
   uint32_t ns = 0, cur = 0xffffffffu;
-  bool ready = false;
   int next_j0 = 0x7fffffff;
   float* out = nullptr;
   const float* planes = nullptr;
@@ -385,7 +424,8 @@
     out = L.out + row * L.stride;
     planes = L.planes + (size_t)v * L.pitch;
   }
-  if (lane == 0) S.ri[warp] = RoundInfo{0, 0, 0, M_IDLE};
+  if (lane < RING) S.ri[lane][warp] = RoundInfo{0, 0, 0, M_IDLE, 0u};
+  if (lane == 0) S.dead_j[warp] = INT_MAX;
   __syncthreads();
   const int c1 = L.chunk0 + min(L.chunk_frames, L.frames - L.chunk0);
   int j = L.chunk0;
@@ -393,58 +433,57 @@
   int pj = -1;
 #pragma unroll
   for (int q = 0; q < V::NPL; q++) pn[q] = 0.0f;
-  for (unsigned rnd_idx = 0;; rnd_idx++) {
-    const bool more = alive && j < c1;
-    bool work = false;
-    int nl = 0;
-    float p[V::NPL];
-#pragma unroll
-    for (int q = 0; q < V::NPL; q++) p[q] = 0.0f;
-    if (more) {
+  typename C::Carry cr{};
+  int last = -DEPTH;
+  bool gen_wait = false;
+  for (unsigned t = 0;; t++) {
+    C::template s_half<NV>(S, warp, lane, t, L.rc);
+    __syncthreads();
+    C::template p_half<NV>(S, warp, lane, t, cr, out, L.rc);
+    const bool drained = last + DEPTH <= (int)t;
+    if (gen_wait && drained) { j += S.ri[(unsigned)last & (RING - 1)][warp].nv; gen_wait = false; }
+    __syncwarp();
+    if (lane == 0) S.ri[t & (RING - 1)][warp] = RoundInfo{j, 0, 0, M_IDLE, 0u};
+    if (alive && !gen_wait && j < c1 && (j != next_j0 || drained)) {
       while (j == next_j0) {
         cur += 1u;
-        if (lane == 0) V::span_begin(a, spans[cur], run, L.rc.sr);
+        if (lane == 0) { V::span_begin(a, spans[cur], run, L.rc.sr); S.dead_j[warp] = INT_MAX; }
         __syncwarp();
-        ready = false;
         next_j0 = cur + 1u < ns ? spans[cur + 1u].j0 : 0x7fffffff;
       }
       const int span_end = min(next_j0, c1);
-      const int act_end = min(span_end, C::active_end(run));
-      if (cur == 0xffffffffu || !V::is_active(a, run, j) || j >= act_end) {
+      if (cur == 0xffffffffu || !V::is_active(a, run, j)) {
         for (int k = j + lane; k < span_end; k += 32) out[k] = 0.0f;
         j = span_end;
       } else {
-        if (!ready) { __syncwarp(); C::span_setup(S, warp, lane, L.rc); __syncwarp(); ready = true; }
-        nl = min(32, act_end - j);
+        const int nl = min(32, span_end - j);
+        float p[V::NPL];
         if (pj == j) {
 #pragma unroll
-          for (int q = 0; q < V::NPL; q++) { const float t = __shfl_sync(FULL, pn[q], nl - 1); p[q] = lane < nl ? pn[q] : t; }
+          for (int q = 0; q < V::NPL; q++) { const float x = __shfl_sync(FULL, pn[q], nl - 1); p[q] = lane < nl ? pn[q] : x; }
         } else {
           const int jj = j + min(lane, nl - 1);
 #pragma unroll
           for (int q = 0; q < V::NPL; q++) p[q] = planes[(size_t)q * L.plane_stride + (jj - L.chunk0)];
         }
-        work = true;
-        pj = j + nl;
-        if (pj < c1) {
-          const int jn = min(pj + lane, c1 - 1);
-#pragma unroll
-          for (int q = 0; q < V::NPL; q++) pn[q] = planes[(size_t)q * L.plane_stride + (jn - L.chunk0)];
-        }
-      }
-    }
-    __syncwarp();
-    if (lane == 0) S.ri[warp] = RoundInfo{j, nl, nl, work ? M_NORMAL : M_IDLE};
-    if (!__syncthreads_or(more ? 1 : 0)) break;
-    float y = 0.0f;
-    int nout = nl;
-    C::template round<NV>(S, warp, lane, work, p, j, nout, y, L.rc, rnd_idx);
-    if (work) {
-      if (lane < nout) out[j + lane] = y;
-      j += nout;
-    }
-  }
-  __syncthreads();
+        int mode = M_IDLE;
+        const int nv = C::template stage_a<NV>(S, warp, lane, t, p, j, nl, drained, cr, mode, L.rc);
+        if (nv >= 0) {
+          pj = j + nl;
+          if (pj < c1) {
+            const int jn = min(pj + lane, c1 - 1);
+#pragma unroll
+            for (int q = 0; q < V::NPL; q++) pn[q] = planes[(size_t)q * L.plane_stride + (jn - L.chunk0)];
+          }
+          if (mode != M_IDLE) last = (int)t;
+          if (mode == M_GENERIC) gen_wait = true;
+          else j += nv;
+        }
+      }
+    }
+    const bool busy = (alive && j < c1) || last + DEPTH > (int)t;
+    if (!__syncthreads_or(busy ? 1 : 0)) break;
+  }
   if (alive) {
     const uint32_t* aw = reinterpret_cast<const uint32_t*>(&a);
     for (int w = lane; w < WA; w += 32) L.state[(size_t)(WC + w) * L.n_pad + sv] = aw[w];
diff --git a/libgooey_b200/csrc/gooey_b200.cu b/libgooey_b200/csrc/gooey_b200.cu
--- a/libgooey_b200/csrc/gooey_b200.cu
+++ b/libgooey_b200/csrc/gooey_b200.cu
@@ -109,13 +109,14 @@
     }
   }
   void launch(cudaStream_t parent, cudaEvent_t start, const gd::RateCtx& rc, const double* tt, int frames, float* out, long long stride) {
-    kicks.launch(parent, start, rc, tt, frames, out, stride);
-    snares.launch(parent, start, rc, tt, frames, out, stride);
-    hats.launch(parent, start, rc, tt, frames, out, stride);
-    toms.launch(parent, start, rc, tt, frames, out, stride);
-    basses.launch(parent, start, rc, tt, frames, out, stride);
-    polys.launch(parent, start, rc, tt, frames, out, stride);
-    grans.launch(parent, start, rc, tt, frames, out, stride);
+    const int drums = kicks.n() + snares.n() + hats.n() + toms.n();
+    kicks.launch(parent, start, rc, tt, frames, out, stride, drums);
+    snares.launch(parent, start, rc, tt, frames, out, stride, drums);
+    hats.launch(parent, start, rc, tt, frames, out, stride, drums);
+    toms.launch(parent, start, rc, tt, frames, out, stride, drums);
+    basses.launch(parent, start, rc, tt, frames, out, stride, drums);
+    polys.launch(parent, start, rc, tt, frames, out, stride, drums);
+    grans.launch(parent, start, rc, tt, frames, out, stride, drums);
   }
   void collect_stats() { kicks.collect_stats(); snares.collect_stats(); hats.collect_stats(); toms.collect_stats(); }
   int chunk_frames(int frames) const { return TypeRunner<gd::KickV>::chunk_of(frames); }
diff --git a/libgooey_b200/csrc/pool.cuh b/libgooey_b200/csrc/pool.cuh
--- a/libgooey_b200/csrc/pool.cuh
+++ b/libgooey_b200/csrc/pool.cuh
@@ -121,12 +121,12 @@
 
 enum class Back { Wave, Coop, Serial };
 constexpr int COOP_FROM = 4096;
-constexpr int COOP_NV = 16;
+constexpr int COOP_NV = 8;
 constexpr int SERIAL_FROM = 12288;
 inline bool serial_backend() { const char* e = getenv("GOOEY_B200_BACKEND"); return e && strcmp(e, "serial") == 0; }
-template <class V> inline Back choose_back(int cnt) {
+template <class V> inline Back choose_back(int cnt, int drums) {
   if (serial_backend()) return Back::Serial;
-  if (std::is_same<V, gd::TomV>::value) return cnt >= COOP_FROM ? Back::Coop : Back::Wave;
+  if (std::is_same<V, gd::TomV>::value) return drums >= COOP_FROM ? Back::Coop : Back::Wave;
   return cnt >= SERIAL_FROM ? Back::Serial : Back::Wave;
 }
 template <class V> struct WaveOf;
@@ -136,7 +136,7 @@
 template <> struct WaveOf<gd::TomV> { using W = gd::wave::TomW; static constexpr const char* name = "wave_kernel<TomW>"; };
 
 inline void coop_launch(int cnt, cudaStream_t s, const gd::VoiceLaunch& L) {
-  using SM = gd::coop::Smem<gd::coop::TomC, COOP_NV>;
+  using SM = gd::coop::TomC::Smem<COOP_NV>;
   auto kernel = gd::coop::coop_kernel<gd::coop::TomC, COOP_NV>;
   static std::mutex mu;
   static std::set<int> done;
@@ -234,7 +234,7 @@
     }
     launched_chunks = -launched_chunks;
   }
-  void launch(cudaStream_t parent, cudaEvent_t start, const gd::RateCtx& rc, const double* tt, int frames, float* out, long long stride) {
+  void launch(cudaStream_t parent, cudaEvent_t start, const gd::RateCtx& rc, const double* tt, int frames, float* out, long long stride, int drums) {
     const int cnt = n();
     launched_chunks = 0;
     if (cnt == 0 || frames <= 0) return;
@@ -278,7 +278,7 @@
       g_launches.fetch_add(1, std::memory_order_relaxed);
       GH_CUDA(cudaGetLastError());
       GH_CUDA(cudaEventRecord(evDoneS, sS));
-      const Back back = choose_back<V>(cnt);
+      const Back back = choose_back<V>(cnt, drums);
       int i = 0;
       for (int c0 = 0; c0 < frames; c0 += chunk, i++) {
         const int b = i & 1;
```

Result: faster. 8.753 billion, median of 6 (+4.2%).
